# da03/torch-Attention-OCR

Measured on AMD Instinct MI355X. Metric: image-lines/sec (train step), higher is better.
Workload: dtype bf16; 1 GPU; c3: 32x256 crops, batch 256/GPU, VGG-7 + BiLSTM(256) + 2-layer attn decoder, L=24; global_batch=256, per_gpu_batch=256, img=32x256, decoder_steps=24, parallelism=dp1, input_feed=True

## Files before the change

### include/aocr.h

```cpp
#ifndef AOCR_H
#define AOCR_H
#include <stddef.h>
#include <stdint.h>

#ifdef __cplusplus
extern "C" {
#endif

#define AOCR_VERSION 1
#define AOCR_NUM_GROUPS 5
#define AOCR_COMPUTE_F32 0
#define AOCR_COMPUTE_BF16 1

typedef struct aocr_model aocr_model;

typedef struct aocr_config {
  int32_t batch_size;
  int32_t img_h;
  int32_t max_img_w;
  int32_t enc_hidden;
  int32_t enc_layers;
  int32_t dec_layers;
  int32_t vocab;
  int32_t emb;
// ... 66 lines not shown
                     const aocr_trie* trie, int32_t* labels_dev, float* scores_dev,
                     float* gold_scores_dev, float* loss_dev);

int aocr_recognize(aocr_model* m, const float* images_dev, int32_t B, int32_t W, int32_t beam,
                   const aocr_trie* trie, int32_t* labels_dev, float* scores_dev,
                   float* char_logp_dev, float* attn_dev);

int aocr_get_tensor(aocr_model* m, const char* name, const void** ptr_dev, int32_t* ndim, int64_t shape[4]);

#define AOCR_PK_CONV6_FWD 0
#define AOCR_PK_CONV6_WGRAD 1
#define AOCR_PK_CONV1_FWD 2
#define AOCR_PK_CONV1_BWD 3
#define AOCR_PK_BN_FWD 4
#define AOCR_PK_BN_BWD 5
#define AOCR_PK_UNPOOL 6
#define AOCR_PK_ATTN_DCTX 7
#define AOCR_PK_SPLITK 8
#define AOCR_PK_LAST 8
int aocr_profile_kernel(aocr_model* m, int32_t which, int32_t iters, float* ms_per_launch, double* flops_per_launch);

#define AOCR_PROF_OTHER 0
#define AOCR_PROF_CONV_FWD 1
#define AOCR_PROF_CONV_DGRAD 2
#define AOCR_PROF_CONV_WGRAD 3
#define AOCR_PROF_BN 4
#define AOCR_PROF_POOL_CONV1 5
#define AOCR_PROF_ENC_SEQ 6
#define AOCR_PROF_RNN_GEMM 7
#define AOCR_PROF_DEC_FWD 8
#define AOCR_PROF_DEC_BWD 9
#define AOCR_PROF_SGD 10
#define AOCR_PROF_DECODE 11
#define AOCR_PROF_FAMILIES 12
int aocr_profile_enable(aocr_model* m, int32_t on);
int aocr_profile_read(aocr_model* m, float ms[AOCR_PROF_FAMILIES], int32_t* marks);


#define AOCR_GEMM_ACCUMULATE 1
#define AOCR_GEMM_RELU 2
#define AOCR_GEMM_TANH 4
int aocr_gemm(void* stream, int32_t compute, const float* A_dev, int64_t lda, int32_t a_kmajor,
              const float* B_dev, int64_t ldb, int32_t b_kmajor, float* C_dev, int64_t ldc,
              int32_t M, int32_t N, int32_t K, const float* bias_dev, int32_t accumulate);

int aocr_conv2d_forward(void* stream, int32_t compute, const float* x_dev, const float* w_dev, const float* bias_dev,
                        float* y_dev, uint8_t* idx_dev, int32_t B, int32_t H, int32_t W, int32_t Cin, int32_t Cout,
                        int32_t ksize, int32_t pad, int32_t relu, int32_t pool);
int aocr_conv2d_backward_data(void* stream, int32_t compute, const float* dy_dev, const float* w_dev, float* dx_dev,
                              int32_t B, int32_t H, int32_t W, int32_t Cin, int32_t Cout, int32_t ksize, int32_t pad);
int aocr_conv2d_backward_filter(void* stream, int32_t compute, const float* x_dev, const float* dy_dev, float* dw_dev,
                                float* dbias_dev, int32_t B, int32_t H, int32_t W, int32_t Cin, int32_t Cout,
                                int32_t ksize, int32_t pad);
int aocr_unpool_relu_backward(void* stream, const float* dpooled_dev, const float* pooled_dev, const uint8_t* idx_dev,
                              float* dy_dev, int32_t B, int32_t Ho, int32_t Wo, int32_t C, int32_t pool);

int aocr_conv1_forward(void* stream, const float* x_dev, const float* w_dev, const float* bias_dev, float* y_dev,
                       int32_t B, int32_t H, int32_t W);
int aocr_conv1_backward(void* stream, const float* x_dev, const float* w_dev, const float* bias_dev,
                        const float* dy_pooled_dev, float* dw_dev, float* dbias_dev, int32_t B, int32_t H, int32_t W);

#define AOCR_BN_SCRATCH_BYTES (8u << 20)
int aocr_batchnorm_relu_forward(void* stream, const float* x_dev, float* y_dev, const float* weight_dev,
                                const float* bias_dev, float* running_mean_dev, float* running_var_dev,
                                float* save_dev, void* scratch_dev, int64_t rows, int32_t C, int32_t training,
                                int32_t update_running, int32_t tb_rows);
int aocr_batchnorm_relu_backward(void* stream, const float* x_dev, const float* y_dev, const float* dA_dev,
                                 const float* weight_dev, const float* save_dev, float* dx_dev, float* dweight_dev,
                                 float* dbias_dev, void* scratch_dev, int64_t rows, int32_t C, int32_t tb_rows);

int aocr_lstm_cell_forward(void* stream, int32_t compute, const float* x_dev, int32_t in_size, const float* h_prev_dev,
                           const float* c_prev_dev, const float* w_i2h_dev, const float* b_i2h_dev,
                           const float* w_h2h_dev, const float* b_h2h_dev, float* c_dev, float* h_dev,
                           float* gates_dev, int32_t B, int32_t H);
int aocr_lstm_cell_forward_zx(void* stream, int32_t compute, const float* zx_dev, int64_t ldzx, const float* h_prev_dev,
                              const float* c_prev_dev, const float* w_h2h_dev, float* c_dev, float* h_dev, float* gates_dev,
                              int32_t B, int32_t H);
int aocr_lstm_cell_backward(void* stream, const float* dc_dev, const float* dh_dev, const float* gates_dev,
                            const float* c_prev_dev, const float* c_dev, float* dz_dev, float* dc_prev_dev,
                            int32_t B, int32_t H);

int aocr_attention_forward(void* stream, const float* ctx_dev, const float* q_dev, float* a_dev, float* c_dev,
                           int64_t ldc, int32_t B, int32_t T, int32_t Hd);
int aocr_attention_backward(void* stream, const float* ctx_dev, const float* q_dev, const float* a_dev,
                            const float* dc_dev, int64_t lddc, float* ds_dev, float* dq_dev, int32_t B, int32_t T,
                            int32_t Hd);

#define AOCR_PW_ADD 0
#define AOCR_PW_TANH_BWD 1
#define AOCR_PW_RELU_BWD 2
#define AOCR_PW_RELU 3
int aocr_pointwise(void* stream, int32_t op, const float* a_dev, const float* b_dev, float* y_dev, int64_t n);

int aocr_lookup_forward(void* stream, const float* weight_dev, const int32_t* ids_dev, float* out_dev, int32_t n, int32_t E);
int aocr_lookup_backward(void* stream, const float* grad_out_dev, const int32_t* ids_dev, float* grad_weight_dev, int32_t n, int32_t E, int32_t V);

int aocr_logsoftmax_nll(void* stream, const float* logits_dev, int64_t ld, const int32_t* targets_dev, float* logp_dev,
                        float* dlogits_dev, float* nll_rows_dev, int64_t rows, int32_t V, float grad_scale);

int aocr_beam_select(void* stream, const float* logp_dev, const int32_t* prev_tok_dev, float* beam_scores_dev,
                     int32_t* tokens_dev, int32_t* parents_dev, int32_t B, int32_t kin, int32_t kout, int32_t V);

int aocr_beam_select_dict(void* stream, const float* logp_dev, const int32_t* prev_tok_dev, float* beam_scores_dev,
                          int32_t* tokens_dev, int32_t* parents_dev, int32_t B, int32_t kin, int32_t kout, int32_t V,
                          const aocr_trie* trie, const int32_t* loc_in_dev, int32_t* loc_out_dev);

// ... 139 lines not shown
```

### torch-attention-ocr_amd/aocr/_lib.py

```python
from __future__ import annotations

import ctypes as C
import os

import torch

_HERE = os.path.dirname(os.path.abspath(__file__))
LIB_PATH = os.environ.get("AOCR_LIB") or os.path.join(_HERE, "libaocr.so")

NUM_GROUPS = 5
COMPUTE_F32, COMPUTE_BF16 = 0, 1
PROF_FAMILIES = ["other", "conv_fwd", "conv_dgrad", "conv_wgrad", "bn", "pool_conv1", "encoder_seq", "rnn_gemm", "decoder_fwd",
                 "decoder_bwd", "sgd", "decode_chain"]


class AocrError(RuntimeError):
    pass


class TrieDesc(C.Structure):
    _fields_ = [("child_mask_dev", C.c_void_p), ("child_base_dev", C.c_void_p), ("child_dev", C.c_void_p),
                ("n_nodes", C.c_int32), ("n_edges", C.c_int32)]


# ... 54 lines not shown
class Config(C.Structure):
    _fields_ = [(n, C.c_int32) for n in (
        "batch_size", "img_h", "max_img_w", "enc_hidden", "enc_layers", "dec_layers", "vocab", "emb",
        "input_feed", "max_decoder_l", "max_beam", "compute")]


if not os.path.exists(LIB_PATH):
    raise ImportError(
        f"{LIB_PATH} not found: build it with `make -C torch-attention-ocr_amd/csrc` "
        "(or __graft_entry__.build()); there is no CPU fallback for the hot path")

lib = C.CDLL(LIB_PATH)

_vp, _i32, _i64, _f32, _sz = C.c_void_p, C.c_int32, C.c_int64, C.c_float, C.c_size_t
_cfgp = C.POINTER(Config)
ALLREDUCE_FN = C.CFUNCTYPE(C.c_int, _vp, _vp, _i64, _i32, _vp)

SIGNATURES = {
    "aocr_last_error": (C.c_char_p, []),
    "aocr_version": (C.c_int, []),
    "aocr_param_counts": (C.c_int, [_cfgp, C.POINTER(_i64)]),
    "aocr_param_entry": (C.c_int, [_cfgp, _i32, C.c_char_p, C.POINTER(_i32), C.POINTER(_i64), C.POINTER(_i32), C.POINTER(_i64)]),
    "aocr_bn_state_count": (_i64, []),
    "aocr_workspace_bytes": (_sz, [_cfgp]),
    "aocr_model_create": (C.c_int, [_cfgp, _vp, _vp, _vp, _vp, _sz, _vp, C.POINTER(_vp)]),
    "aocr_model_destroy": (C.c_int, [_vp]),
    "aocr_model_set_stream": (C.c_int, [_vp, _vp]),
    "aocr_train_forward_backward": (C.c_int, [_vp, _vp, _vp, _vp, _i32, _i32, _i32, _f32, _vp]),
    "aocr_set_dropout": (C.c_int, [_vp, C.c_double, C.c_uint64, C.c_uint64]),
    "aocr_cluster_status": (C.c_int, [_vp, C.POINTER(_i32)]),
    "aocr_grad_buckets": (C.c_int, [_cfgp, C.POINTER(_i64), C.POINTER(_i64)]),
    "aocr_stream_wait_grads": (C.c_int, [_vp, _i32, _vp]),
    "aocr_comm_unique_id": (C.c_int, [C.c_char_p]),
    "aocr_comm_init_rank": (C.c_int, [_vp, C.c_char_p, _i32, _i32, _i32]),
    "aocr_comm_set_callback": (C.c_int, [_vp, _vp, _vp, _i32, _i32]),
    "aocr_allreduce_grads": (C.c_int, [_vp, _vp]),
    "aocr_comm_destroy": (C.c_int, [_vp]),
    "aocr_comm_exposed_ms": (C.c_int, [_vp, C.POINTER(_f32)]),
    "aocr_comm_info": (C.c_int, [_vp, C.POINTER(_i32), C.POINTER(_i32), C.POINTER(_i32)]),
    "aocr_sgd_step": (C.c_int, [_vp, _f32, _f32, _vp]),
    "aocr_adadelta_step": (C.c_int, [_vp, _f32, _f32, _f32, _vp]),
    "aocr_forward_logits": (C.c_int, [_vp, _vp, _vp, _vp, _i32, _i32, _i32, _i32, _vp, _vp]),
    "aocr_decode": (C.c_int, [_vp, _vp, _vp, _vp, _i32, _i32, _i32, _i32, _vp, _vp, _vp, _vp]),
    "aocr_decode_dict": (C.c_int, [_vp, _vp, _vp, _vp, _i32, _i32, _i32, _i32, _vp, _vp, _vp, _vp, _vp]),
    "aocr_recognize": (C.c_int, [_vp, _vp, _i32, _i32, _i32, _vp, _vp, _vp, _vp, _vp]),
    "aocr_get_tensor": (C.c_int, [_vp, C.c_char_p, C.POINTER(_vp), C.POINTER(_i32), C.POINTER(_i64)]),
    "aocr_profile_kernel": (C.c_int, [_vp, _i32, _i32, C.POINTER(_f32), C.POINTER(C.c_double)]),
    "aocr_profile_enable": (C.c_int, [_vp, _i32]),
    "aocr_profile_read": (C.c_int, [_vp, C.POINTER(_f32), C.POINTER(_i32)]),
    "aocr_gemm": (C.c_int, [_vp, _i32, _vp, _i64, _i32, _vp, _i64, _i32, _vp, _i64, _i32, _i32, _i32, _vp, _i32]),
    "aocr_conv2d_forward": (C.c_int, [_vp, _i32, _vp, _vp, _vp, _vp, _vp] + [_i32] * 9),
    "aocr_conv2d_backward_data": (C.c_int, [_vp, _i32, _vp, _vp, _vp] + [_i32] * 7),
    "aocr_conv2d_backward_filter": (C.c_int, [_vp, _i32, _vp, _vp, _vp, _vp] + [_i32] * 7),
    "aocr_unpool_relu_backward": (C.c_int, [_vp, _vp, _vp, _vp, _vp] + [_i32] * 5),
    "aocr_conv1_forward": (C.c_int, [_vp, _vp, _vp, _vp, _vp, _i32, _i32, _i32]),
    "aocr_conv1_backward": (C.c_int, [_vp, _vp, _vp, _vp, _vp, _vp, _vp, _i32, _i32, _i32]),
    "aocr_batchnorm_relu_forward": (C.c_int, [_vp] * 9 + [_i64, _i32, _i32, _i32, _i32]),
    "aocr_batchnorm_relu_backward": (C.c_int, [_vp] * 10 + [_i64, _i32, _i32]),
    "aocr_lstm_cell_forward": (C.c_int, [_vp, _i32, _vp, _i32] + [_vp] * 9 + [_i32, _i32]),
    "aocr_lstm_cell_forward_zx": (C.c_int, [_vp, _i32, _vp, _i64] + [_vp] * 6 + [_i32, _i32]),
    "aocr_lstm_cell_backward": (C.c_int, [_vp] * 8 + [_i32, _i32]),
    "aocr_attention_forward": (C.c_int, [_vp, _vp, _vp, _vp, _vp, _i64, _i32, _i32, _i32]),
    "aocr_attention_backward": (C.c_int, [_vp, _vp, _vp, _vp, _vp, _i64, _vp, _vp, _i32, _i32, _i32]),
    "aocr_pointwise": (C.c_int, [_vp, _i32, _vp, _vp, _vp, _i64]),
    "aocr_lookup_forward": (C.c_int, [_vp, _vp, _vp, _vp, _i32, _i32]),
    "aocr_lookup_backward": (C.c_int, [_vp, _vp, _vp, _vp, _i32, _i32, _i32]),
    "aocr_logsoftmax_nll": (C.c_int, [_vp, _vp, _i64, _vp, _vp, _vp, _vp, _i64, _i32, _f32]),
    "aocr_beam_select_dict": (C.c_int, [_vp, _vp, _vp, _vp, _vp, _vp, _i32, _i32, _i32, _i32, _vp, _vp, _vp]),
    "aocr_edit_distance": (C.c_int, [_vp, _vp, _vp, _i32, _i32, _vp, _vp]),
    "aocr_lexicon_scratch_bytes": (_sz, [_i32, _i32]),
    "aocr_lexicon_nearest": (C.c_int, [_vp, _vp, _i32, _i32, _vp, _vp, _vp, _vp, _vp]),
    "aocr_preprocess_lines": (C.c_int, [_vp, _vp, _vp, _i32, _i32, _i32, _vp]),
    "aocr_augment_lines": (C.c_int, [_vp, _vp, _vp, _i32, _i32, _i32, C.c_uint64, C.c_uint64, _vp]),
    "aocr_synth_lines": (C.c_int, [_vp, _vp, _vp, _vp, _i32, _i32, _i32, _i32, _vp, _vp, _vp]),
    "aocr_segment_scratch_bytes": (C.c_size_t, [_i32, _i32, _i32]),
    "aocr_segment_page": (C.c_int, [_vp, _vp, C.c_int64, _i32, _i32, _vp, _vp, _i32, _vp, _vp]),
    "aocr_crop_lines": (C.c_int, [_vp, _vp, C.c_int64, _i32, _i32, _vp, _vp, _i32, _i32, _i32, _vp]),
    "aocr_skew_scratch_bytes": (C.c_size_t, [_i32, _i32, _i32]),
    "aocr_estimate_skew": (C.c_int, [_vp, _vp, C.c_int64, _i32, _i32, _vp, _vp, _vp, _vp]),
    "aocr_deskew_page": (C.c_int, [_vp, _vp, C.c_int64, _i32, _i32, _vp, _i32, _i32, _vp, C.c_int64]),
    "aocr_flatten_scratch_bytes": (C.c_size_t, [_i32, _i32, _i32]),
    "aocr_flatten_page": (C.c_int, [_vp, _vp, C.c_int64, _i32, _i32, _vp, _vp, _vp, C.c_int64]),
    "aocr_integral_scratch_bytes": (C.c_size_t, [_i32, _i32]),
    "aocr_ink_integral": (C.c_int, [_vp, _vp, C.c_int64, _i32, _i32, _i32, _i32, _vp, _vp, C.c_int64, _vp]),
    "aocr_layout_scratch_bytes": (C.c_size_t, [_i32, _i32, _i32]),
    "aocr_layout_blocks": (C.c_int, [_vp, _vp, C.c_int64, _i32, _i32, _vp, _vp, _i32, _vp, _vp]),
    "aocr_components_scratch_bytes": (C.c_size_t, [_i32, _i32]),
    "aocr_label_components": (C.c_int, [_vp, _vp, C.c_int64, _i32, _i32, _i32, _i32, _i32, _vp, _vp, C.c_int64, _i32, _vp, _vp]),
    "aocr_clean_scratch_bytes": (C.c_size_t, [_i32, _i32]),
    "aocr_clean_page": (C.c_int, [_vp, _vp, C.c_int64, _i32, _i32, _vp, _vp, _vp, C.c_int64, _vp]),
    "aocr_beam_select": (C.c_int, [_vp, _vp, _vp, _vp, _vp, _vp, _i32, _i32, _i32, _i32]),
}

for _name, (_res, _args) in SIGNATURES.items():
    _fn = getattr(lib, _name)
    _fn.restype = _res
    _fn.argtypes = _args


def last_error() -> str:
    return (lib.aocr_last_error() or b"").decode()


def check(rc: int, what: str = "") -> None:
    if rc != 0:
        raise AocrError(f"{what}: {last_error()}" if what else last_error())
# ... 26 lines not shown
```

### torch-attention-ocr_amd/csrc/capi.hip

```cpp
#include <cmath>
#include <cstdarg>
#include <cstdio>
#include <cstring>
#include <new>
#include <string>
#include "model.h"

using namespace aocr;

static thread_local std::string g_err;
static int fail(const char* fmt, ...) {
  char buf[512]; va_list ap; va_start(ap, fmt); vsnprintf(buf, sizeof buf, fmt, ap); va_end(ap);
  g_err = buf; return 1;
}
static int check_launch(const char* what) {
  hipError_t e = hipGetLastError();
  if (e != hipSuccess) return fail("%s: %s", what, hipGetErrorString(e));
  return 0;
}
#define REQUIRE(cond, ...) do { if (!(cond)) return fail(__VA_ARGS__); } while (0)

static int check_cfg(const aocr_config* c) {
  REQUIRE(c, "config is NULL");
  REQUIRE(c->batch_size >= 1 && c->img_h >= 32 && c->img_h % 16 == 0, "bad batch_size/img_h");
// ... 408 lines not shown
  else if (n == "enc_cs0") { *ptr_dev = m->ecs[0][m->Le - 1]; *ndim = 3; shape[0] = d.T + 2; shape[1] = d.B; shape[2] = m->He; }
  else if (n == "enc_gates0") { *ptr_dev = m->egates[0][m->Le - 1]; *ndim = 3; shape[0] = d.T; shape[1] = d.B; shape[2] = 4 * m->He; }
  else if (n == "cl_err") { *ptr_dev = m->cl_err; *ndim = 1; shape[0] = 8; REQUIRE(m->cl_err, "no cluster kernels in this configuration"); }
  else if (n == "dc_stamps") { REQUIRE(m->dc_xtab, "no decoder cluster kernel in this configuration"); *ptr_dev = m->dc_xtab + (size_t)((d.B + 31) / 32) * 32; *ndim = 1; shape[0] = 32; }
  else if (n == "ds_all") { *ptr_dev = m->ds_all; *ndim = 3; shape[0] = d.L; shape[1] = d.B; shape[2] = d.T; }
  else if (n == "dq_all") { *ptr_dev = m->dq_all; *ndim = 3; shape[0] = d.L; shape[1] = d.B; shape[2] = m->Hd; }
  else if (n == "dcat_all") { *ptr_dev = m->dcat_all; *ndim = 3; shape[0] = d.L; shape[1] = d.B; shape[2] = 2 * m->Hd; }
  else if (n == "dh_rec0" || n == "dh_rec1" || n == "dc_st0" || n == "dc_st1" || n == "dfeed0") {
    const int l = n.back() - '0'; *ptr_dev = n[1] == 'f' ? m->dfeed : (n[1] == 'h' ? m->dh_rec[l] : m->dc_st[l]); *ndim = 2; shape[0] = d.B; shape[1] = m->Hd; }
  else if (n == "dpre_all") { *ptr_dev = m->dpre_all; *ndim = 3; shape[0] = d.L; shape[1] = d.B; shape[2] = m->Hd; }
  else if (n == "dc_bstamps") { REQUIRE(m->dc_xtab, "no decoder cluster kernel in this configuration"); *ptr_dev = m->dc_xtab + (size_t)((d.B + 31) / 32) * 32 + 16; *ndim = 1; shape[0] = 32; }
  else if (n == "dc_times") { REQUIRE(m->cl_err, "no cluster kernels in this configuration"); *ptr_dev = m->cl_err + 16 + 2048; *ndim = 1; shape[0] = 32 * 4 * 16 * 2; }
  else if (n == "g0") {
    const char* e = getenv("AOCR_DBG_STOP"); const int stop = e ? atoi(e) : 0;
    const int64_t cnt = stop == 1 ? (int64_t)d.B * d.T * 512 : (int64_t)d.B * d.H4 * d.W2 * 512;
    if (m->bf16) bf16_to_f32(m->s, m->G0b, m->G0, cnt);
    *ptr_dev = m->G0; *ndim = 4; shape[0] = d.B; shape[1] = stop == 1 ? d.Ho7 : d.H4; shape[2] = stop == 1 ? d.Wo7 : d.W2; shape[3] = 512;
  }
  else return fail("unknown tensor '%s'", name);
  return 0;
}

int aocr_profile_kernel(aocr_model* m, int32_t which, int32_t iters, float* ms_per_launch, double* flops_per_launch) {
  REQUIRE(m && ms_per_launch && flops_per_launch, "NULL argument");
  REQUIRE(m->last_valid, "run a step first");
  REQUIRE(which >= 0 && which <= AOCR_PK_LAST, "unknown kernel id %d", which);
  REQUIRE(iters >= 1, "iters must be >= 1");
  REQUIRE(which < 2 || (m->bf16 && m->last_images && m->last_train), "the HBM-bound kernel ids replay the bf16 TRAINING step: run aocr_train_forward_backward in bf16 mode first");
  const Dims& d = m->last;
  const int64_t n5 = (int64_t)d.B * d.H4 * d.W2;
  REQUIRE((which != 1 && which != AOCR_PK_SPLITK) || (size_t)512 * 4608 <= m->gmax, "kernel id %d sums conv6's filter gradient (512 x 4608 floats) into the gradient-map scratch, which holds %zu floats in this configuration", which, m->gmax);
  REQUIRE((which != AOCR_PK_BN_FWD && which != AOCR_PK_BN_BWD && which != AOCR_PK_UNPOOL) || (n5 % 256 == 0 && n5 / 256 <= 512), "kernel id %d replays conv5's BatchNorm with the epilogue's 256-pixel statistics chunks: %lld pixels are not a multiple of 256 / more than 512 chunks", which, (long long)n5);
  hipEvent_t e0, e1; hipEventCreate(&e0); hipEventCreate(&e1);
  hipStream_t s = m->s; const int B = d.B;
  constexpr size_t SLAB = (size_t)4 << 20;
  double bytes = 0.0;
  const char* const nd = getenv("AOCR_DX16");
  const bool dx16 = (nd && nd[0] == '1') && !getenv("AOCR_BN_PARTIAL_OLD") && !getenv("AOCR_UNPOOL4") && !getenv("AOCR_HALO8") && B * d.H4 * d.W2 % 256 == 0;
  const bf16_t* const g1h = dx16 ? reinterpret_cast<const bf16_t*>(m->G1) : nullptr;
  const double dab = dx16 ? 2.0 : 4.0;
  auto run = [&]() {
    switch (which) {
    case 0:
      if (const char* const pl = getenv("AOCR_PROBE_LAYER")) {
        int bnc = 0, y16 = 0; const int l = atoi(pl);
        if (l == 3) { conv_forward(m->s, m->bf16, m->A2, m->conv[3].w, m->conv[3].b, m->Y3, nullptr, d.B, d.H2, d.W2, 128, 256, 3, 1, 0, 0, m->A2b, m->wb[3], nullptr, 1, nullptr, nullptr, nullptr, (double*)m->bn_scratch, &bnc, &y16); break; }
        if (l == 4) { conv_forward(m->s, m->bf16, m->A3, m->conv[4].w, m->conv[4].b, nullptr, m->idx4, d.B, d.H2, d.W2, 256, 256, 3, 1, 1, 2, m->A3b, m->wb[4], m->A4b, 1); break; }
        if (l == 5) { conv_forward(m->s, m->bf16, m->A4, m->conv[5].w, m->conv[5].b, m->Y5, nullptr, d.B, d.H4, d.W2, 256, 512, 3, 1, 0, 0, m->A4b, m->wb[5], nullptr, 1, nullptr, nullptr, nullptr, (double*)m->bn_scratch, &bnc, &y16); break; }
      }
      conv_forward(m->s, m->bf16, m->A5, m->conv[6].w, m->conv[6].b, m->bf16 ? nullptr : m->A6, m->idx6, d.B, d.H4, d.W2, 512, 512, 3, 1, 1, 2, m->A5b, m->wb[6],
                   m->A6b, 1);
      break;
    case 1:
      conv_backward_filter(m->s, m->bf16, m->A5, m->G0, m->G1, nullptr, d.B, d.H4, d.W2, 512, 512, 3, 1, m->A5b, m->G0b, m->wg_part, m->wg_part_floats, 1);
      break;
    case AOCR_PK_CONV1_FWD:
      conv1_forward(s, m->last_images, m->conv[1].w, m->conv[1].b, nullptr, B, d.H, d.W, m->A1b, m->route1_valid ? m->route1 : nullptr);
      bytes = (double)B * d.H * d.W * 4 + (double)B * d.H1 * d.W1 * 64 * 2 + (m->route1_valid ? (double)conv1_route_elems(B, d.H, d.W) * 2 : 0.0);
      break;
    case AOCR_PK_CONV1_BWD:
      conv1_backward(s, m->last_images, m->conv[1].w, m->conv[1].b, m->G1, m->conv[1].dw, m->conv[1].db, B, d.H, d.W,
                     (size_t)B * d.H1 * d.W1 * 128 >= (size_t)4096 * 640 ? m->G0 + 6 * SLAB : nullptr, nullptr, m->route1_valid ? m->route1 : nullptr);
      bytes = (double)B * d.H * d.W * 4 + (double)B * d.H1 * d.W1 * 64 * 4 + (m->route1_valid ? (double)conv1_route_elems(B, d.H, d.W) * 2 : 0.0);
      break;
    case AOCR_PK_BN_FWD:
      bn_relu_forward(s, m->Y5, nullptr, m->bn[5].w, m->bn[5].b, m->bn[5].rm, m->bn[5].rv, m->bn[5].save, m->bn_scratch, n5, 512, 1, 0, 0, m->A5b, nullptr, (int)(n5 / 256));
      bytes = (double)n5 * 512 * (4 + 2);
      break;
    case AOCR_PK_BN_BWD:
      bn_relu_backward(s, m->Y5, m->A5, m->G1, m->bn[5].w, m->bn[5].save, nullptr, m->bn[5].dw, m->bn[5].db, m->bn_scratch, n5, 512, 0, m->G0b, m->A5b,
                       m->conv[5].db, m->G0 + 2 * SLAB, nullptr, nullptr, nullptr, g1h);
      bytes = (double)n5 * 512 * ((4 + dab + 2) + (4 + dab + 2 + 2));
      break;
    case AOCR_PK_UNPOOL:
      unpool_relu_backward(s, m->G1, m->A6, m->idx6, nullptr, B, d.H4, d.W2, 512, 2, m->G0b, m->conv[6].db, m->G0 + 1 * SLAB, m->A6b, nullptr, g1h);
      bytes = (double)B * d.H6 * d.W2 * 512 * (dab + 1 + 2) + (double)n5 * 512 * 2;
      break;
    case AOCR_PK_ATTN_DCTX:
      attention_dctx(s, m->a_all, m->ds_all, m->dcat_all, 2 * m->Hd, m->q_all, m->dctx, d.L, B, d.T, m->Hd);
      bytes = (double)d.L * B * (2.0 * d.T + 2.0 * m->Hd) * 4 + (double)B * d.T * m->Hd * 4;
      break;
    case AOCR_PK_SPLITK:
      {
        const int ksl = (int)std::min<size_t>(8, m->wg_part_floats / ((size_t)512 * 4608));
        if (ksl >= 1) splitk_reduce(s, m->wg_part, ksl, (size_t)512 * 4608, m->G1);
        bytes = (double)512 * 4608 * 4 * (ksl + 2);
      }
      break;
    }
  };
  run();
  hipEventRecord(e0, m->s);
  for (int i = 0; i < iters; ++i) run();
  hipEventRecord(e1, m->s);
  hipEventSynchronize(e1);
  float ms = 0.f; hipEventElapsedTime(&ms, e0, e1);
  hipEventDestroy(e0); hipEventDestroy(e1);
  *ms_per_launch = ms / iters;
  if (which == 0 && getenv("AOCR_PROBE")) {
    unsigned long long pr[8] = {0}; kprobe_read(pr);
    if (getenv("AOCR_PROBE_LAYER")) for (int k = 1; k >= 0; --k) if (pr[4 * k + 1]) fprintf(stderr, "[aocr] probe: workgroup %d of the tagged launch: start -> K loop %.1f us, K loop %.1f us (%llu cycles = %.2f GHz), whole workgroup (last store acknowledged) %.1f us\n", k ? 17 : 300, pr[4 * k + 2] / 100.0, pr[4 * k + 1] / 100.0, pr[4 * k], pr[4 * k] / (pr[4 * k + 1] * 10.0) , pr[4 * k + 3] / 100.0);
    for (int k = 0; k < 2; ++k) if (pr[4 * k + 1]) fprintf(stderr, "[aocr] probe (%s halo kernel, conv6 forward): K loop of one workgroup %llu shader cycles in %.1f us = %.2f GHz\n", k ? "4-wave" : "8-wave", pr[4 * k], pr[4 * k + 1] / 100.0, pr[4 * k] / (pr[4 * k + 1] * 10.0)), fprintf(stderr, "[aocr]   prologue %.1f us, whole workgroup %.1f us (stores acknowledged)\n", pr[4 * k + 2] / 100.0, pr[4 * k + 3] / 100.0);
  }
  *flops_per_launch = which < 2 ? 2.0 * (double)d.B * d.H4 * d.W2 * 512.0 * (9.0 * 512.0) : bytes;
  return check_launch("aocr_profile_kernel");
}

int aocr_gemm(void* stream, int32_t compute, const float* A_dev, int64_t lda, int32_t a_kmajor, const float* B_dev, int64_t ldb,
              int32_t b_kmajor, float* C_dev, int64_t ldc, int32_t M, int32_t N, int32_t K, const float* bias_dev, int32_t accumulate) {
  REQUIRE(A_dev && B_dev && C_dev && M >= 0 && N >= 0 && K >= 0, "bad gemm arguments");
  REQUIRE((accumulate & ~7) == 0, "unknown gemm flag bits %d", accumulate);
  const int fl = ((accumulate & AOCR_GEMM_ACCUMULATE) ? EP_ACCUM : 0) | ((accumulate & AOCR_GEMM_RELU) ? EP_RELU : 0) | ((accumulate & AOCR_GEMM_TANH) ? EP_TANH : 0);
  REQUIRE(!((fl & EP_ACCUM) && (fl & (EP_RELU | EP_TANH))), "an activation on an accumulating product is not a module of the path");
  int rc = gemm((hipStream_t)stream, compute == AOCR_COMPUTE_BF16, A_dev, lda, a_kmajor != 0, B_dev, ldb, b_kmajor != 0, C_dev, ldc,
                M, N, K, bias_dev, nullptr, fl);
  REQUIRE(rc == 0, "gemm: the (A column-major, B row-major-by-K) combination is not supported");
  return check_launch("aocr_gemm");
}
int aocr_pointwise(void* stream, int32_t op, const float* a_dev, const float* b_dev, float* y_dev, int64_t n) {
  REQUIRE(a_dev && y_dev && n >= 0 && op >= 0 && op <= 3 && (b_dev || op == AOCR_PW_RELU), "bad arguments");
  pointwise((hipStream_t)stream, op, a_dev, b_dev, y_dev, n);
  return check_launch("aocr_pointwise");
}
int aocr_lookup_forward(void* stream, const float* weight_dev, const int32_t* ids_dev, float* out_dev, int32_t n, int32_t E) {
  REQUIRE(weight_dev && ids_dev && out_dev && n >= 0 && E > 0, "bad arguments");
  embedding_gather((hipStream_t)stream, weight_dev, ids_dev, 0, 1, out_dev, 1, n, E);
  return check_launch("aocr_lookup_forward");
}
int aocr_lookup_backward(void* stream, const float* grad_out_dev, const int32_t* ids_dev, float* grad_weight_dev, int32_t n, int32_t E, int32_t V) {
  REQUIRE(grad_out_dev && ids_dev && grad_weight_dev && n >= 0 && E > 0 && E <= 256 && V > 0, "bad arguments");
  embedding_scatter_accum((hipStream_t)stream, grad_out_dev, ids_dev, 0, 1, grad_weight_dev, 1, n, E, V);
  return check_launch("aocr_lookup_backward");
}
int aocr_conv2d_forward(void* stream, int32_t compute, const float* x_dev, const float* w_dev, const float* bias_dev, float* y_dev,
                        uint8_t* idx_dev, int32_t B, int32_t H, int32_t W, int32_t Cin, int32_t Cout, int32_t ksize, int32_t pad,
                        int32_t relu, int32_t pool) {
  REQUIRE(x_dev && w_dev && y_dev, "NULL argument");
  REQUIRE(Cin % 16 == 0 && Cout % 16 == 0, "Cin and Cout must be multiples of 16 (the 1-channel first layer has its own entry point)");
  REQUIRE(pool >= 0 && pool <= 2 && (pool == 0 || idx_dev), "bad pool mode / missing idx");
  conv_forward((hipStream_t)stream, compute == AOCR_COMPUTE_BF16, x_dev, w_dev, bias_dev, y_dev, idx_dev, B, H, W, Cin, Cout, ksize, pad,
               relu, pool);
  return check_launch("aocr_conv2d_forward");
}
int aocr_conv2d_backward_data(void* stream, int32_t compute, const float* dy_dev, const float* w_dev, float* dx_dev, int32_t B, int32_t H,
                              int32_t W, int32_t Cin, int32_t Cout, int32_t ksize, int32_t pad) {
  REQUIRE(dy_dev && w_dev && dx_dev && Cin % 16 == 0 && Cout % 16 == 0, "bad arguments");
  conv_backward_data((hipStream_t)stream, compute == AOCR_COMPUTE_BF16, dy_dev, w_dev, dx_dev, B, H, W, Cin, Cout, ksize, pad);
  return check_launch("aocr_conv2d_backward_data");
}
int aocr_conv2d_backward_filter(void* stream, int32_t compute, const float* x_dev, const float* dy_dev, float* dw_dev, float* dbias_dev,
                                int32_t B, int32_t H, int32_t W, int32_t Cin, int32_t Cout, int32_t ksize, int32_t pad) {
  REQUIRE(x_dev && dy_dev && dw_dev && Cin % 16 == 0 && Cout % 16 == 0, "bad arguments");
  conv_backward_filter((hipStream_t)stream, compute == AOCR_COMPUTE_BF16, x_dev, dy_dev, dw_dev, dbias_dev, B, H, W, Cin, Cout, ksize, pad);
  return check_launch("aocr_conv2d_backward_filter");
}
int aocr_unpool_relu_backward(void* stream, const float* dpooled_dev, const float* pooled_dev, const uint8_t* idx_dev, float* dy_dev,
                              int32_t B, int32_t Ho, int32_t Wo, int32_t C, int32_t pool) {
  REQUIRE(dpooled_dev && pooled_dev && idx_dev && dy_dev && (pool == 1 || pool == 2) && C % 4 == 0, "bad arguments");
  unpool_relu_backward((hipStream_t)stream, dpooled_dev, pooled_dev, idx_dev, dy_dev, B, Ho, Wo, C, pool);
  return check_launch("aocr_unpool_relu_backward");
}
int aocr_conv1_forward(void* stream, const float* x_dev, const float* w_dev, const float* bias_dev, float* y_dev, int32_t B, int32_t H,
                       int32_t W) {
  REQUIRE(x_dev && w_dev && bias_dev && y_dev, "NULL argument");
  conv1_forward((hipStream_t)stream, x_dev, w_dev, bias_dev, y_dev, B, H, W);
  return check_launch("aocr_conv1_forward");
}
int aocr_conv1_backward(void* stream, const float* x_dev, const float* w_dev, const float* bias_dev, const float* dy_pooled_dev,
                        float* dw_dev, float* dbias_dev, int32_t B, int32_t H, int32_t W) {
  REQUIRE(x_dev && w_dev && bias_dev && dy_pooled_dev && dw_dev && dbias_dev, "NULL argument");
  conv1_backward((hipStream_t)stream, x_dev, w_dev, bias_dev, dy_pooled_dev, dw_dev, dbias_dev, B, H, W);
  return check_launch("aocr_conv1_backward");
}
int aocr_batchnorm_relu_forward(void* stream, const float* x_dev, float* y_dev, const float* weight_dev, const float* bias_dev,
                                float* running_mean_dev, float* running_var_dev, float* save_dev, void* scratch_dev, int64_t rows,
                                int32_t C, int32_t training, int32_t update_running, int32_t tb_rows) {
  REQUIRE(x_dev && y_dev && weight_dev && bias_dev && running_mean_dev && running_var_dev && save_dev && scratch_dev, "NULL argument");
  REQUIRE(C % 4 == 0 && C <= 512, "C must be a multiple of 4 and <= 512");
  bn_relu_forward((hipStream_t)stream, x_dev, y_dev, weight_dev, bias_dev, running_mean_dev, running_var_dev, save_dev, scratch_dev, rows, C,
                  training, update_running, tb_rows);
  return check_launch("aocr_batchnorm_relu_forward");
}
int aocr_batchnorm_relu_backward(void* stream, const float* x_dev, const float* y_dev, const float* dA_dev, const float* weight_dev,
                                 const float* save_dev, float* dx_dev, float* dweight_dev, float* dbias_dev, void* scratch_dev,
                                 int64_t rows, int32_t C, int32_t tb_rows) {
  REQUIRE(x_dev && y_dev && dA_dev && weight_dev && save_dev && dx_dev && dweight_dev && dbias_dev && scratch_dev, "NULL argument");
  bn_relu_backward((hipStream_t)stream, x_dev, y_dev, dA_dev, weight_dev, save_dev, dx_dev, dweight_dev, dbias_dev, scratch_dev, rows, C,
                   tb_rows);
  return check_launch("aocr_batchnorm_relu_backward");
}
int aocr_lstm_cell_forward(void* stream, int32_t compute, const float* x_dev, int32_t in_size, const float* h_prev_dev,
                           const float* c_prev_dev, const float* w_i2h_dev, const float* b_i2h_dev, const float* w_h2h_dev,
                           const float* b_h2h_dev, float* c_dev, float* h_dev, float* gates_dev, int32_t B, int32_t H) {
  REQUIRE(x_dev && h_prev_dev && c_prev_dev && w_i2h_dev && b_i2h_dev && w_h2h_dev && b_h2h_dev && c_dev && h_dev, "NULL argument");
  REQUIRE(in_size % 16 == 0 && H % 16 == 0, "in_size and H must be multiples of 16");
  GatesFwdArgs z;
  z.a = make_loadk2(x_dev, in_size, in_size, h_prev_dev, H, H, B);
  z.b = make_loadk2(w_i2h_dev, in_size, in_size, w_h2h_dev, H, H, 4 * H);
  z.K = in_size + H;
  EpGatesFwd& e = z.ep; e.zx = nullptr; e.ldzx = 0; e.b1 = b_i2h_dev; e.b2 = b_h2h_dev; e.c_prev = c_prev_dev; e.ldcp = H;
  e.c_out = c_dev; e.ldc = H; e.h_out = h_dev; e.ldh = H; e.h_out2 = nullptr; e.ldh2 = 0; e.gates = gates_dev; e.ldg = 4 * H; e.M = B; e.H = H;
  launch_small_gates_fwd((hipStream_t)stream, compute == AOCR_COMPUTE_BF16, 1, &z, B, H);
  return check_launch("aocr_lstm_cell_forward");
}
int aocr_lstm_cell_forward_zx(void* stream, int32_t compute, const float* zx_dev, int64_t ldzx, const float* h_prev_dev, const float* c_prev_dev,
                              const float* w_h2h_dev, float* c_dev, float* h_dev, float* gates_dev, int32_t B, int32_t H) {
  REQUIRE(zx_dev && h_prev_dev && c_prev_dev && w_h2h_dev && c_dev && h_dev, "NULL argument");
  REQUIRE(H % 16 == 0 && ldzx >= 4 * (int64_t)H, "H must be a multiple of 16 and ldzx >= 4H");
// ... 347 lines not shown
```

### torch-attention-ocr_amd/csrc/mfma_gemm.h

```cpp
#pragma once
#include <hip/hip_runtime.h>
#include <stdint.h>
#include <type_traits>
#include <utility>

namespace aocr {

typedef float f32x16 __attribute__((ext_vector_type(16)));
typedef float f32x4 __attribute__((ext_vector_type(4)));
typedef __bf16 bf16x8 __attribute__((ext_vector_type(8)));

template <int NV> struct Frag { float v[NV]; };

template <bool BF16> struct Mode {
  static constexpr int NV = BF16 ? 8 : 4;
  static constexpr int CHUNK = BF16 ? 16 : 8;
};


struct LoadK {
  const float* p0; int64_t ld0; int K0;
  const float* p1; int64_t ld1;
  int rows; int K; int vec;
  struct Ctx { const float* b0; const float* b1; bool ok; };
// ... 1834 lines not shown
#pragma unroll
  for (int i = 0; i < 2; ++i)
#pragma unroll
    for (int j = 0; j < 2; ++j)
#pragma unroll
      for (int e = 0; e < 16; ++e) acc[i][j][e] = 0.f;

  const int g = lane >> 4, q = (lane >> 2) & 3, p = lane & 3;
  const int tr_off = (8 * h + q) * TR_PITCH + (16 * (g & 1) + 4 * p) * 2;

  if (nk > 0) { gload(); lwrite(0); }
  __syncthreads();
  for (int kt = 0; kt < nk; ++kt) {
    const int buf = kt & 1;
    if (kt + 1 < nk) gload();
    const unsigned char* la = &lds[buf][0][tr_off + (wm * 64) * 2];
    const unsigned char* lb = &lds[buf][1][tr_off + (wn * 64) * 2];
#pragma unroll
    for (int s = 0; s < 2; ++s) {
      bf16x8 af[2], bf[2];
#pragma unroll
      for (int i = 0; i < 2; ++i) {
        s16x4 a0 = lds_tr_read(la + (16 * s) * TR_PITCH + i * 64), a1 = lds_tr_read(la + (16 * s + 4) * TR_PITCH + i * 64);
        s16x4 b0 = lds_tr_read(lb + (16 * s) * TR_PITCH + i * 64), b1 = lds_tr_read(lb + (16 * s + 4) * TR_PITCH + i * 64);
        typedef short s16x8 __attribute__((ext_vector_type(8)));
        s16x8 av = {a0[0], a0[1], a0[2], a0[3], a1[0], a1[1], a1[2], a1[3]};
        s16x8 bv = {b0[0], b0[1], b0[2], b0[3], b1[0], b1[1], b1[2], b1[3]};
        af[i] = __builtin_bit_cast(bf16x8, av); bf[i] = __builtin_bit_cast(bf16x8, bv);
      }
#pragma unroll
      for (int mi = 0; mi < 2; ++mi)
#pragma unroll
        for (int ni = 0; ni < 2; ++ni)
          acc[mi][ni] = __builtin_amdgcn_mfma_f32_32x32x16_bf16(af[mi], bf[ni], acc[mi][ni], 0, 0, 0);
    }
    if (kt + 1 < nk) lwrite(buf ^ 1);
    __syncthreads();
  }
  const int r = lane & 31;
  const int m0 = m_blk + wm * 64, n0 = n_blk + wn * 64;
#pragma unroll
  for (int mi = 0; mi < 2; ++mi)
#pragma unroll
    for (int qq = 0; qq < 4; ++qq) {
      float v[2][4];
#pragma unroll
      for (int ni = 0; ni < 2; ++ni)
#pragma unroll
        for (int i = 0; i < 4; ++i) v[ni][i] = acc[mi][ni][4 * qq + i];
      ep.template quad<2>(m0 + 32 * mi + 8 * qq + 4 * h, n0 + r, 32, v);
    }
}

template <class EP>
__global__ __launch_bounds__(256, 4) void conv_wgrad_tr_kernel(LoadMNh a, LoadConvXcolh b, EP ep, int K, int kper, int gx, int gy, int gz, float* part, long long pstride) {
  __shared__ __attribute__((aligned(16))) unsigned char lds[2][2][32 * TR_PITCH];
  const int nwg = gx * gy * gz, orig = blockIdx.x;
  const int q8 = nwg >> 3, r8 = nwg & 7, xcd = orig & 7;
  const int lin = (xcd < r8 ? xcd * (q8 + 1) : r8 * (q8 + 1) + (xcd - r8) * q8) + (orig >> 3);
  const int zsp = lin / (gx * gy), bid = lin - zsp * (gx * gy);
  const int kbeg = zsp * kper;
  if (part) { ep.C = part + (size_t)zsp * pstride; ep.flags &= ~8 ; }
  tr_tile(a, b, ep, (bid / gx) * 128, (bid % gx) * 128, kbeg, min(K, kbeg + kper), lds);
}

template <class EP, int ABL = 0>
__global__ __launch_bounds__(512, 1) void conv_wgrad_dma_kernel(LoadMNh a, LoadConvXcolh b, EP ep, int K, int kper, int gx, int gy, const bf16_t* zero, int gz, float* part, long long pstride) {
  __shared__ __attribute__((aligned(1024))) unsigned char lds[4 * 32768];
  const int nwg = gx * gy * gz, orig = blockIdx.x;
  const int q8 = nwg >> 3, r8 = nwg & 7, xcd = orig & 7;
  const int lin = (xcd < r8 ? xcd * (q8 + 1) : r8 * (q8 + 1) + (xcd - r8) * q8) + (orig >> 3);
  const int zsp = lin / (gx * gy), bid = lin - zsp * (gx * gy);
  const int m_blk = (bid / gx) * 256, n_blk = (bid % gx) * 256;
  const int kbeg = zsp * kper, kend = min(K, kbeg + kper);
  if (part) { ep.C = part + (size_t)zsp * pstride; ep.flags &= ~8 ; }
  const int nk = kend > kbeg ? (kend - kbeg + 31) >> 5 : 0;
  const int tid = threadIdx.x, lane = tid & 63, wave = __builtin_amdgcn_readfirstlane(tid >> 6);
  const int h = lane >> 5, wm = wave >> 2, wn = wave & 3;

  int krow[2], chunk[2];
#pragma unroll
  for (int j = 0; j < 2; ++j) {
    krow[j] = 2 * (2 * wave + j) + (lane >> 5);
    const int pos = lane & 31;
    chunk[j] = ((((pos >> 2) ^ (krow[j] & 3)) << 2) | (pos & 3));
  }
  LoadMNh::Ctx8 ca[2]; typename LoadConvXcolh::Ctx8 cb[2]; typename LoadConvXcolh::Cur cur[2]; int ka[2];
#pragma unroll
  for (int j = 0; j < 2; ++j) {
    ca[j] = a.row8(m_blk + 8 * chunk[j]); cb[j] = b.row8(n_blk + 8 * chunk[j]);
    cur[j] = b.seek(cb[j], kbeg + krow[j]); ka[j] = kbeg + krow[j];
  }
  const bf16_t* pa[2]; const int64_t astep = 32 * a.ld;
#pragma unroll
  for (int j = 0; j < 2; ++j) pa[j] = ca[j].b + (int64_t)ka[j] * a.ld;
  unsigned char* const wbase = lds + (2 * wave) * 1024;
  int slot = 0;
  auto issue = [&]() {
#pragma unroll
    for (int j = 0; j < 2; ++j) {
      dma16((ABL & 16) ? zero : dma_select(ca[j].ok && ka[j] < kend, pa[j], zero), wbase + slot * 32768 + j * 1024);
      ka[j] += 32; pa[j] += astep;
    }
#pragma unroll
    for (int j = 0; j < 2; ++j) {
      dma16((ABL & 128) ? zero : b.dsrc8(cb[j], cur[j], kend, zero), wbase + slot * 32768 + 16384 + j * 1024);
      b.advance(cb[j], cur[j]);
    }
    slot = (slot + 1) & 3;
  };

  f32x16 acc[4][2];
#pragma unroll
  for (int i = 0; i < 4; ++i)
#pragma unroll
    for (int j = 0; j < 2; ++j)
#pragma unroll
      for (int e = 0; e < 16; ++e) acc[i][j][e] = 0.f;

  const int g = lane >> 4, q = (lane >> 2) & 3, p4 = lane & 3;
  const unsigned rowoff = (8 * h + q) * 512 + (16 * (g & 1) + 4 * p4) * 2;
  unsigned aseg[4], bseg[2];
#pragma unroll
  for (int i = 0; i < 4; ++i) aseg[i] = rowoff + (((wm * 4 + i) ^ q) << 6);
#pragma unroll
  for (int i = 0; i < 2; ++i) bseg[i] = 16384 + rowoff + (((wn * 2 + i) ^ q) << 6);

  typedef unsigned long long u64;
  typedef u64 u64x2 __attribute__((ext_vector_type(2)));
  const unsigned lbase = (unsigned)(uintptr_t)((__attribute__((address_space(3))) unsigned char*)lds);
#define AOCR_TRR(dst, addr, OFF) asm volatile("ds_read_b64_tr_b16 %0, %1 offset:" #OFF : "=v"(dst) : "v"(addr))
#pragma unroll
  for (int t = 0; t < 3; ++t) issue();
  for (int kt = 0; kt < nk; ++kt) {
    asm volatile("s_waitcnt vmcnt(8)" ::: "memory");
    __builtin_amdgcn_s_barrier();
    const unsigned sl = lbase + (kt & 3) * 32768;
    u64 fa[2][4][2], fb[2][2][2];
#pragma unroll
    for (int i = 0; i < 4; ++i) {
      const unsigned ad = sl + aseg[i];
      if constexpr (ABL & 4) { fa[0][i][0] = fa[0][i][1] = fa[1][i][0] = fa[1][i][1] = ad; continue; }
      AOCR_TRR(fa[0][i][0], ad, 0); AOCR_TRR(fa[0][i][1], ad, 2048); AOCR_TRR(fa[1][i][0], ad, 8192); AOCR_TRR(fa[1][i][1], ad, 10240);
    }
#pragma unroll
    for (int i = 0; i < 2; ++i) {
      const unsigned ad = sl + bseg[i];
      if constexpr (ABL & 4) { fb[0][i][0] = fb[0][i][1] = fb[1][i][0] = fb[1][i][1] = ad; continue; }
      AOCR_TRR(fb[0][i][0], ad, 0); AOCR_TRR(fb[0][i][1], ad, 2048); AOCR_TRR(fb[1][i][0], ad, 8192); AOCR_TRR(fb[1][i][1], ad, 10240);
    }
    if constexpr (!(ABL & 1)) issue();
    asm volatile("s_waitcnt lgkmcnt(0)"
                 : "+v"(fa[0][0][0]), "+v"(fa[0][0][1]), "+v"(fa[0][1][0]), "+v"(fa[0][1][1]), "+v"(fa[0][2][0]), "+v"(fa[0][2][1]),
                   "+v"(fa[0][3][0]), "+v"(fa[0][3][1]), "+v"(fb[0][0][0]), "+v"(fb[0][0][1]), "+v"(fb[0][1][0]), "+v"(fb[0][1][1])
                 :: "memory");
    asm volatile(""
                 : "+v"(fa[1][0][0]), "+v"(fa[1][0][1]), "+v"(fa[1][1][0]), "+v"(fa[1][1][1]), "+v"(fa[1][2][0]), "+v"(fa[1][2][1]),
                   "+v"(fa[1][3][0]), "+v"(fa[1][3][1]), "+v"(fb[1][0][0]), "+v"(fb[1][0][1]), "+v"(fb[1][1][0]), "+v"(fb[1][1][1])
                 :: "memory");
#pragma unroll
    for (int s2 = 0; s2 < 2; ++s2)
#pragma unroll
      for (int mi = 0; mi < 4; ++mi)
#pragma unroll
        for (int ni = 0; ni < 2; ++ni) {
          const u64x2 av = {fa[s2][mi][0], fa[s2][mi][1]}, bv = {fb[s2][ni][0], fb[s2][ni][1]};
          if constexpr (ABL & 2) { acc[mi][ni][0] += (float)(unsigned)(av[0] ^ bv[1]); continue; }
          acc[mi][ni] = __builtin_amdgcn_mfma_f32_32x32x16_bf16(__builtin_bit_cast(bf16x8, av), __builtin_bit_cast(bf16x8, bv), acc[mi][ni], 0, 0, 0);
        }
  }
#undef AOCR_TRR
  asm volatile("s_waitcnt vmcnt(0) lgkmcnt(0)" ::: "memory");
  const int r = lane & 31;
  const int m0 = m_blk + wm * 128, n0 = n_blk + wn * 64;
  if constexpr (std::is_same<EP, EpStore>::value && ABL == 0) {
    if (part && !ep.flags && !ep.bias && !ep.bias2 && !ep.C1 && !ep.Cb && !ep.dg && m_blk + 256 <= ep.M && n_blk + 256 <= ep.N) {
      tile256_store_f32<2, 512>(ep.C, ep.ldc, nullptr, false, acc, lds, m_blk, n_blk, wm, wn, r, h, tid);
      return;
    }
  }
#pragma unroll
  for (int mi = 0; mi < 4; ++mi)
#pragma unroll
    for (int qq = 0; qq < 4; ++qq) {
      float v[2][4];
#pragma unroll
      for (int ni = 0; ni < 2; ++ni)
#pragma unroll
        for (int i = 0; i < 4; ++i) v[ni][i] = acc[mi][ni][4 * qq + i];
      ep.template quad<2>(m0 + 32 * mi + 8 * qq + 4 * h, n0 + r, 32, v);
    }
}

struct WgDmaProblem { const bf16_t* A; const bf16_t* B; long long lda, ldb; int M, N, K, gx, tiles, ks, kper, first; float* part; float* C; long long ldc; long long f4first; };
struct WgDmaArgs { int n, total; long long f4total; WgDmaProblem p[8]; };
template <int UNUSED = 0>
__global__ __launch_bounds__(512, 1) void wgrad_dma_grouped_kernel(WgDmaArgs g, const bf16_t* zero) {
  __shared__ __attribute__((aligned(1024))) unsigned char lds[4 * 32768];
  int pi = 0;
#pragma unroll
  for (int i = 1; i < 8; ++i) if (i < g.n && (int)blockIdx.x >= g.p[i].first) pi = i;
  const WgDmaProblem& P = g.p[pi];
  const int local = blockIdx.x - P.first;
  const int zsp = local / P.tiles, bid = local - zsp * P.tiles;
  const int m_blk = (bid / P.gx) * 256, n_blk = (bid % P.gx) * 256;
  const int kbeg = zsp * P.kper, kend = min(P.K, kbeg + P.kper);
  const int nk = kend > kbeg ? (kend - kbeg + 31) >> 5 : 0;
  const int tid = threadIdx.x, lane = tid & 63, wave = __builtin_amdgcn_readfirstlane(tid >> 6);
  const int h = lane >> 5, wm = wave >> 2, wn = wave & 3;
  const bf16_t* pa[2]; const bf16_t* pb[2]; int ka[2];
#pragma unroll
  for (int j = 0; j < 2; ++j) {
    const int krow = 2 * (2 * wave + j) + (lane >> 5), pos = lane & 31;
    const int chunk = ((((pos >> 2) ^ (krow & 3)) << 2) | (pos & 3));
    ka[j] = kbeg + krow;
    pa[j] = P.A + (long long)ka[j] * P.lda + m_blk + 8 * chunk; pb[j] = P.B + (long long)ka[j] * P.ldb + n_blk + 8 * chunk;
  }
  const long long astep = 32 * P.lda, bstep = 32 * P.ldb;
  unsigned char* const wbase = lds + (2 * wave) * 1024;
  int slot = 0;
  auto issue = [&]() {
#pragma unroll
    for (int j = 0; j < 2; ++j) { dma16(dma_select(ka[j] < kend, pa[j], zero), wbase + slot * 32768 + j * 1024); pa[j] += astep; }
#pragma unroll
    for (int j = 0; j < 2; ++j) { dma16(dma_select(ka[j] < kend, pb[j], zero), wbase + slot * 32768 + 16384 + j * 1024); pb[j] += bstep; ka[j] += 32; }
    slot = (slot + 1) & 3;
  };
  f32x16 acc[4][2];
#pragma unroll
  for (int i = 0; i < 4; ++i)
#pragma unroll
    for (int j = 0; j < 2; ++j)
#pragma unroll
      for (int e = 0; e < 16; ++e) acc[i][j][e] = 0.f;
  const int gq = lane >> 4, q = (lane >> 2) & 3, p4 = lane & 3;
  const unsigned rowoff = (8 * h + q) * 512 + (16 * (gq & 1) + 4 * p4) * 2;
  unsigned aseg[4], bseg[2];
#pragma unroll
  for (int i = 0; i < 4; ++i) aseg[i] = rowoff + (((wm * 4 + i) ^ q) << 6);
#pragma unroll
  for (int i = 0; i < 2; ++i) bseg[i] = 16384 + rowoff + (((wn * 2 + i) ^ q) << 6);
  typedef unsigned long long u64;
  typedef u64 u64x2 __attribute__((ext_vector_type(2)));
  const unsigned lbase = (unsigned)(uintptr_t)((__attribute__((address_space(3))) unsigned char*)lds);
// ... 11 lines not shown
      AOCR_TRR(fa[0][i][0], ad, 0); AOCR_TRR(fa[0][i][1], ad, 2048); AOCR_TRR(fa[1][i][0], ad, 8192); AOCR_TRR(fa[1][i][1], ad, 10240);
    }
#pragma unroll
    for (int i = 0; i < 2; ++i) {
      const unsigned ad = sl + bseg[i];
      AOCR_TRR(fb[0][i][0], ad, 0); AOCR_TRR(fb[0][i][1], ad, 2048); AOCR_TRR(fb[1][i][0], ad, 8192); AOCR_TRR(fb[1][i][1], ad, 10240);
    }
    issue();
    asm volatile("s_waitcnt lgkmcnt(0)"
                 : "+v"(fa[0][0][0]), "+v"(fa[0][0][1]), "+v"(fa[0][1][0]), "+v"(fa[0][1][1]), "+v"(fa[0][2][0]), "+v"(fa[0][2][1]),
                   "+v"(fa[0][3][0]), "+v"(fa[0][3][1]), "+v"(fb[0][0][0]), "+v"(fb[0][0][1]), "+v"(fb[0][1][0]), "+v"(fb[0][1][1])
                 :: "memory");
    asm volatile(""
                 : "+v"(fa[1][0][0]), "+v"(fa[1][0][1]), "+v"(fa[1][1][0]), "+v"(fa[1][1][1]), "+v"(fa[1][2][0]), "+v"(fa[1][2][1]),
                   "+v"(fa[1][3][0]), "+v"(fa[1][3][1]), "+v"(fb[1][0][0]), "+v"(fb[1][0][1]), "+v"(fb[1][1][0]), "+v"(fb[1][1][1])
                 :: "memory");
#pragma unroll
    for (int s2 = 0; s2 < 2; ++s2)
#pragma unroll
      for (int mi = 0; mi < 4; ++mi)
#pragma unroll
        for (int ni = 0; ni < 2; ++ni) {
          const u64x2 av = {fa[s2][mi][0], fa[s2][mi][1]}, bv = {fb[s2][ni][0], fb[s2][ni][1]};
          acc[mi][ni] = __builtin_amdgcn_mfma_f32_32x32x16_bf16(__builtin_bit_cast(bf16x8, av), __builtin_bit_cast(bf16x8, bv), acc[mi][ni], 0, 0, 0);
        }
  }
#undef AOCR_TRR
  asm volatile("s_waitcnt vmcnt(0) lgkmcnt(0)" ::: "memory");
  tile256_store_f32<2, 512>(P.part + (size_t)zsp * P.M * P.N, P.N, nullptr, false, acc, lds, m_blk, n_blk, wm, wn, lane & 31, h, tid);
}
template <int UNUSED = 0>
__global__ __launch_bounds__(256) void wgrad_slab_reduce_kernel(WgDmaArgs g) {
  typedef float f4 __attribute__((ext_vector_type(4)));
  const long long i = (long long)blockIdx.x * 256 + threadIdx.x;
  if (i >= g.f4total) return;
  int pi = 0;
#pragma unroll
  for (int k = 1; k < 8; ++k) if (k < g.n && i >= g.p[k].f4first) pi = k;
  const WgDmaProblem& P = g.p[pi];
  const long long li = i - P.f4first; const int n4 = P.N >> 2; const long long m = li / n4; const int c = (int)(li - m * n4) * 4;
  const size_t mn = (size_t)P.M * P.N;
  const float* src = P.part + (size_t)m * P.N + c;
  f4 acc = {0.f, 0.f, 0.f, 0.f};
  for (int z = 0; z < P.ks; ++z) acc += __builtin_nontemporal_load(reinterpret_cast<const f4*>(src + (size_t)z * mn));
  float* o = P.C + m * P.ldc + c;
  o[0] += acc[0]; o[1] += acc[1]; o[2] += acc[2]; o[3] += acc[3];
}

template <int... I, class F> __device__ __forceinline__ void aocr_static_for_impl(std::integer_sequence<int, I...>, F&& f) { (f(std::integral_constant<int, I>{}), ...); }
template <int N, class F> __device__ __forceinline__ void aocr_static_for(F&& f) { aocr_static_for_impl(std::make_integer_sequence<int, N>{}, f); }
template <int TAG = 0, int MG = 4, bool RG = false, bool IM = false>
__global__ __launch_bounds__(128 * MG, 1)
void conv_wgrad_halo_kernel(const bf16_t* __restrict__ dy, const bf16_t* __restrict__ x, float* __restrict__ part, long long pstride,
                            int nimg, int H, int W, int Cin, int Cout, int gx, int gy, int gz, int segs_per, const bf16_t* zero) {
  constexpr int MT = 64 * MG, NWV = 2 * MG, AROW = MT * 2, RPP = 1024 / AROW, LPR = 64 / RPP;
  constexpr int BOFF = 32 * AROW, SLOT = BOFF + 8192, NS = 6, PW = 34, HPW = 8 / NWV;
  __shared__ __attribute__((aligned(1024))) unsigned char lds[NWV * 20480 > NS * SLOT ? NWV * 20480 : NS * SLOT];
  const int nwg = gx * gy * gz, orig = blockIdx.x;
  const int q8 = nwg >> 3, r8 = nwg & 7, xcd = orig & 7;
  const int lin = (xcd < r8 ? xcd * (q8 + 1) : r8 * (q8 + 1) + (xcd - r8) * q8) + (orig >> 3);
  const int zsp = lin / (gx * gy), bid = lin - zsp * (gx * gy);
  const int m_blk = (bid / gx) * MT, cchunk = bid % gx;
  const int spr = (W + 31) >> 5, S = nimg * H * spr;
  const int s_beg = zsp * segs_per, s_end = min(S, s_beg + segs_per);
  const int nk = s_end > s_beg ? s_end - s_beg : 0;
  const int tid = threadIdx.x, lane = tid & 63, wave = __builtin_amdgcn_readfirstlane(tid >> 6);
  const int h = lane >> 5, mg = wave & (MG - 1), tg = wave / MG;

  const int wrap_px = W - 32 * (spr - 1);
  const int64_t seg0_px = (int64_t)(s_beg / spr) * W + 32 * (s_beg % spr);
  const bf16_t* pa[2]; int akrow[2];
#pragma unroll
  for (int j = 0; j < 2; ++j) {
    const int krow = RPP * (2 * wave + j) + lane / LPR, pos = lane & (LPR - 1);
    const int chunk = ((((pos >> 2) ^ (krow & 3)) << 2) | (pos & 3));
    akrow[j] = krow;
    pa[j] = dy + (seg0_px + krow) * Cout + m_blk + 8 * chunk;
  }
  const int64_t astep = (int64_t)32 * Cout, awrap = (int64_t)wrap_px * Cout;
  bool bin[HPW]; int bry[HPW], bcx[HPW]; const bf16_t* pb[HPW];
#pragma unroll
  for (int j = 0; j < HPW; ++j) {
    const int sl = 64 * (HPW * wave + j) + lane;
    bin[j] = sl < 3 * PW * 4;
    const int hry = sl / (PW * 4), hrem = sl - hry * (PW * 4), hcx = hrem >> 2, hc = hrem & 3;
    bry[j] = hry - 1; bcx[j] = hcx - 1;
    pb[j] = x + (seg0_px + (int64_t)(hry - 1) * W + (hcx - 1)) * Cin + cchunk * 32 + hc * 8;
  }
  const int64_t bstep = (int64_t)32 * Cin, bwrap = (int64_t)wrap_px * Cin;
  int is = s_beg, ixs = s_beg % spr, iy = (s_beg / spr) % H;
  unsigned char* const wA = lds + (2 * wave) * 1024;
  unsigned char* const wB = lds + BOFF + (HPW * wave) * 1024;
  int islot = 0;
  auto issue = [&]() {
    const bool live = is < s_end;
    const int x0 = ixs << 5;
    if constexpr (RG) {
      const bool last = ixs + 1 == spr;
#pragma unroll
      for (int j = 0; j < 2; ++j) { dma16(dma_select(live && x0 + akrow[j] < W, pa[j], zero), wA + islot * SLOT + j * 1024); pa[j] += last ? awrap : astep; }
#pragma unroll
      for (int j = 0; j < HPW; ++j) {
        const bool ok = live && bin[j] && (unsigned)(iy + bry[j]) < (unsigned)H && (unsigned)(x0 + bcx[j]) < (unsigned)W;
        dma16(dma_select(ok, pb[j], zero), wB + islot * SLOT + j * 1024); pb[j] += last ? bwrap : bstep;
      }
      ++is; if (last) { ixs = 0; if (++iy == H) iy = 0; } else ++ixs;
    } else {
// ... 54 lines not shown
            const u64x2 av = {fa[s2][mi][0], fa[s2][mi][1]}, bv = {fb[s2][t][0], fb[s2][t][1]};
            acc[mi][t] = __builtin_amdgcn_mfma_f32_32x32x16_bf16(__builtin_bit_cast(bf16x8, av), __builtin_bit_cast(bf16x8, bv), acc[mi][t], 0, 0, 0);
          }
      };
      if constexpr (!IM) {
        issue();
        asm volatile("s_waitcnt lgkmcnt(0)" : "+v"(fa[0][0][0]), "+v"(fa[0][0][1]), "+v"(fa[0][1][0]), "+v"(fa[0][1][1]), "+v"(fa[1][0][0]), "+v"(fa[1][0][1]), "+v"(fa[1][1][0]), "+v"(fa[1][1][1]) :: "memory");
#pragma unroll
        for (int s2 = 0; s2 < 2; ++s2)
#pragma unroll
          for (int t = 0; t < NTP; ++t) asm volatile("" : "+v"(fb[s2][t][0]), "+v"(fb[s2][t][1]));
        mma_half(std::integral_constant<int, 0>{}); mma_half(std::integral_constant<int, 1>{});
      } else {
        asm volatile("s_waitcnt lgkmcnt(%4)" : "+v"(fa[0][0][0]), "+v"(fa[0][0][1]), "+v"(fa[0][1][0]), "+v"(fa[0][1][1]) : "n"(4 + 2 * NTP) : "memory");
#pragma unroll
        for (int t = 0; t < NTP; ++t) asm volatile("" : "+v"(fb[0][t][0]), "+v"(fb[0][t][1]));
        __builtin_amdgcn_sched_barrier(0);
        mma_half(std::integral_constant<int, 0>{});
        __builtin_amdgcn_sched_barrier(0);
        issue();
        __builtin_amdgcn_sched_barrier(0);
        asm volatile("s_waitcnt lgkmcnt(0)" : "+v"(fa[1][0][0]), "+v"(fa[1][0][1]), "+v"(fa[1][1][0]), "+v"(fa[1][1][1]) :: "memory");
#pragma unroll
        for (int t = 0; t < NTP; ++t) asm volatile("" : "+v"(fb[1][t][0]), "+v"(fb[1][t][1]));
        mma_half(std::integral_constant<int, 1>{});
      }
    }
    asm volatile("s_waitcnt vmcnt(0) lgkmcnt(0)" ::: "memory");
    __syncthreads();
    unsigned char* const wl = lds + wave * 20480;
    constexpr int RP = NTP * 128;
#pragma unroll
    for (int mi = 0; mi < 2; ++mi) {
#pragma unroll
      for (int t = 0; t < NTP; ++t)
#pragma unroll
        for (int qq = 0; qq < 4; ++qq)
#pragma unroll
          for (int i = 0; i < 4; ++i)
            *reinterpret_cast<float*>(wl + (8 * qq + 4 * h + i) * RP + (t * 32 + r) * 4) = acc[mi][t][4 * qq + i];
      asm volatile("s_waitcnt lgkmcnt(0)" ::: "memory");
      const int co0 = m_blk + mg * 64 + mi * 32;
#pragma unroll 4
      for (int it = 0; it < 4 * NTP; ++it) {
        const int idx = it * 64 + lane, row = idx / (8 * NTP), c4 = idx - row * (8 * NTP), t = c4 >> 3, j = c4 & 7;
        const float4 v = *reinterpret_cast<const float4*>(wl + row * RP + c4 * 16);
        *reinterpret_cast<float4*>(slab + (int64_t)(co0 + row) * ldw + (int64_t)(T0 + t) * Cin + cchunk * 32 + j * 4) = v;
      }
      asm volatile("s_waitcnt lgkmcnt(0)" ::: "memory");
    }
  };
  if (tg == 0) body(std::integral_constant<int, 0>{}); else body(std::integral_constant<int, 1>{});
#undef AOCR_TRH
}

template <class AL, class BL, class EP> struct GroupProblem { AL a; BL b; EP ep; int K, kper, gx, ksplit, first; };
template <class AL, class BL, class EP> struct GroupArgs { int n, total; GroupProblem<AL, BL, EP> p[8]; };

template <class AL, class BL, class EP>
__global__ __launch_bounds__(256) void gemm_lds_grouped_kernel(GroupArgs<AL, BL, EP> g) {
  __shared__ __attribute__((aligned(16))) unsigned char lds[2][2][128 * LDS_PITCH];
  int pi = 0;
#pragma unroll
  for (int i = 1; i < 8; ++i) if (i < g.n && (int)blockIdx.x >= g.p[i].first) pi = i;
  const GroupProblem<AL, BL, EP>& P = g.p[pi];
  const int local = blockIdx.x - P.first;
  const int tile = local / P.ksplit, z = local - tile * P.ksplit;
  const int kbeg = z * P.kper;
  lds_tile<32>(P.a, P.b, P.ep, (tile / P.gx) * 128, (tile % P.gx) * 128, kbeg, min(P.K, kbeg + P.kper), lds);
}
template <class EP>
__global__ __launch_bounds__(256, 4) void wgrad_tr_grouped_kernel(GroupArgs<LoadMNh, LoadMNh, EP> g) {
  __shared__ __attribute__((aligned(16))) unsigned char lds[2][2][32 * TR_PITCH];
  int pi = 0;
#pragma unroll
  for (int i = 1; i < 8; ++i) if (i < g.n && (int)blockIdx.x >= g.p[i].first) pi = i;
  const GroupProblem<LoadMNh, LoadMNh, EP>& P = g.p[pi];
  const int local = blockIdx.x - P.first;
  const int tile = local / P.ksplit, z = local - tile * P.ksplit;
  const int kbeg = z * P.kper;
  tr_tile(P.a, P.b, P.ep, (tile / P.gx) * 128, (tile % P.gx) * 128, kbeg, min(P.K, kbeg + P.kper), lds);
}

template <class AL, class BL, class EP> struct SmallArgs { AL a; BL b; EP ep; int K; };

template <bool BF16, int NT, bool GATES, int NW, bool QG, class AL, class BL, class EP>
__device__ __forceinline__ void gemm_small_body(const SmallArgs<AL, BL, EP>& g, int gate_stride, float* red) {
  constexpr int NV = Mode<BF16>::NV, CH = Mode<BF16>::CHUNK;
  const int lane = threadIdx.x & 63, wave = threadIdx.x >> 6;
  const int r = lane & 31, h = lane >> 5;
  const int m0 = blockIdx.y * 32;
  const int n0 = QG ? blockIdx.x * 8 : (GATES ? blockIdx.x * 32 : blockIdx.x * 32 * NT);
  const int K = g.K;

  typename AL::Ctx ca[1]; typename BL::Ctx cb[NT];
  ca[0] = g.a.row(m0 + r);
#pragma unroll
  for (int i = 0; i < NT; ++i) cb[i] = g.b.row(QG ? (r >> 3) * gate_stride + n0 + (r & 7) : (GATES ? i * gate_stride + n0 + r : n0 + 32 * i + r));

  f32x16 acc[1][NT];
#pragma unroll
  for (int j = 0; j < NT; ++j)
#pragma unroll
    for (int e = 0; e < 16; ++e) acc[0][j][e] = 0.f;

  typedef typename FragOf<AL, NV>::type FA; typedef typename FragOf<BL, NV>::type FB;
// ... 332 lines not shown
```

### torch-attention-ocr_amd/csrc/model.h

```cpp
#pragma once
#include <string>
#include <vector>
#include "../../include/aocr.h"
#include "ops.h"

namespace aocr {

constexpr int MAXL = 4;
constexpr int LOGIT_LD = 40;

struct ParamEntry { std::string name; int group; int64_t offset; int ndim; int64_t shape[4]; int64_t numel; };
struct Layout { std::vector<ParamEntry> e; int64_t group_off[AOCR_NUM_GROUPS + 1]; };
Layout build_layout(const aocr_config& c);

struct ConvP { float *w, *b, *dw, *db; int cin, cout, ks, pad; };
struct BnP { float *w, *b, *dw, *db, *rm, *rv, *save; int C; };
struct ShW { const float* w; int64_t ld; int R, C; bf16_t* wb; bf16_t* wtb; float* wtf; };
struct LstmP { float *wi, *bi, *wh, *bh, *dwi, *dbi, *dwh, *dbh; int in; ShW swi, swh; };

struct Arena {
  char* base; size_t off;
  template <class T> T* get(size_t n) {
    off = (off + 255) & ~(size_t)255;
    T* p = base ? reinterpret_cast<T*>(base + off) : nullptr;
    off += n * sizeof(T);
    return p;
  }
};

struct CommState {
  int nranks = 1; bool sync_bn = false; int provider = 0;
  void* rccl = nullptr; void* rccl_bn = nullptr; aocr_allreduce_fn fn = nullptr; void* user = nullptr;
  hipStream_t stream = nullptr; hipEvent_t done = nullptr;
  hipEvent_t wait0 = nullptr, wait1 = nullptr; bool timed = false;
};

struct Dims {
  int B, H, W, L, T;
  int H1, W1, H2, W2, H4, H6, Ho7, Wo7;
};
bool make_dims(const aocr_config& c, int B, int W, int L, Dims& d);

}

struct aocr_model {
  aocr_config cfg;
  hipStream_t s;
  bool bf16;
  float *params, *grads, *bn_state;
  aocr::Layout layout;
  aocr::ConvP conv[8];
  aocr::BnP bn[8];
  aocr::LstmP enc[2][aocr::MAXL], dec[aocr::MAXL];
  float *lookup, *dlookup, *wa, *dwa, *wc, *dwc, *wo, *bo, *dwo, *dbo;
  aocr::ShW swa, swc;
  int He, Hd, Le, Ld, E, V;

  size_t ws_bytes;
  float *A1, *A2, *Y3, *A3, *A4, *Y5, *A5, *A6, *Y7, *X;
  uint8_t *idx2, *idx4, *idx6;
  uint16_t* route1 = nullptr; bool route1_valid = false;
  float *G0, *G1, *dX; size_t gmax = 0;
  aocr::bf16_t *A1b, *A2b, *A3b, *A4b, *A5b, *A6b, *G0b, *G2b = nullptr;
  hipEvent_t cw_map[2] = {nullptr, nullptr}, cw_done[2] = {nullptr, nullptr}, cw_main = nullptr;
  aocr::bf16_t *wb[8], *wtb[8];
  float* wtf[8];
  aocr::bf16_t *Xb, *ehs_b[2][aocr::MAXL], *edz_b[2][aocr::MAXL], *dhs_b[aocr::MAXL], *ddz_b[aocr::MAXL], *out_b, *cat_b, *dpre_b, *dq_b;
  void* bn_scratch; float* bn_save;
  int y16[2] = {0, 0};
  float *ezx[2][aocr::MAXL], *ehs[2][aocr::MAXL], *ecs[2][aocr::MAXL], *egates[2][aocr::MAXL], *edz[2][aocr::MAXL], *edc[2][aocr::MAXL];
  float *edxl[2];
  float *context, *dctx;
  aocr::bf16_t* context_b;
  float* emb_seg = nullptr; int* emb_index = nullptr; bool emb_table = false, tab_valid = false;
  hipEvent_t tab_done = nullptr, zero_done = nullptr, shadow_done = nullptr, shadow2_done = nullptr; bool tab_ready = false, zero_pending = false, shadow_pending = false, shadow2_pending = false;
  int shadow_tiles_conv2 = 0;
  bool proj_fused = false, dout_ready = false;
  float* loss_pending = nullptr;
  hipEvent_t q_go = nullptr, q_done = nullptr; bool q_pending = false;
  hipEvent_t enc_ev = nullptr;
  float *emb_all, *zx1_all, *dhs[aocr::MAXL], *dcs[aocr::MAXL], *dgates[aocr::MAXL], *ddz[aocr::MAXL];
  float *out_all, *cat_all, *q_all, *a_all, *logits, *dlogits, *nll_rows;
  float *dout_proj, *dpre_all, *dcat_all, *ds_all, *dq_all, *demb_all;
  float *dh_rec[aocr::MAXL], *dc_st[aocr::MAXL], *dfeed, *loss_tmp;
  float *bc[2][aocr::MAXL], *bh[2][aocr::MAXL], *bfeed[2], *bc_new[aocr::MAXL], *bh_new[aocr::MAXL];
  aocr::bf16_t *bh_b[2][aocr::MAXL] = {}, *bfeed_b[2] = {}, *bh_new_b[aocr::MAXL] = {}, *bcat_b = nullptr;
  float *bzx1, *bzx_tab, *bq, *ba, *bcat, *bout, *blogits, *blogp, *beam_scores;
  int32_t *hist_tok, *hist_par, *tgt_pad, *tge_pad, *trie_loc[2];
  float *attn_hist = nullptr, *sc_hist = nullptr;
  void* sgd_scratch;
  float* wg_part = nullptr; size_t wg_part_floats = 0;

  std::vector<aocr::ShadowJob> shadow_host;
  aocr::ShadowJob* shadow_dev; int shadow_tiles;
  hipEvent_t grad_ev[4];
  hipStream_t lay_s[aocr::MAXL] = {}; std::vector<hipEvent_t> lay_ev;
  hipStream_t side2 = nullptr; hipEvent_t side2_done = nullptr;
  hipStream_t side = nullptr; hipEvent_t side_go = nullptr, side_done = nullptr; bool side_busy = false;
  int64_t conv5_off;
  aocr::Dims last;
  int last_valid;
  const float* last_images = nullptr; bool last_train = false;
  unsigned long long *cl_xbuf = nullptr, *cl_pbuf = nullptr, *cl_xtab = nullptr; int* cl_err = nullptr; size_t cl_xbytes = 0, cl_pbytes = 0, cl_tbytes = 0; unsigned cl_epoch = 0;
  unsigned long long *dc_xbuf = nullptr, *dc_xtab = nullptr; size_t dc_xbytes = 0, dc_tbytes = 0; aocr::bf16_t* ctxa_b = nullptr; bool ctxa_fresh = false;  bool dgates_il = false; unsigned long long* dc_bxbuf = nullptr; size_t dc_bxbytes = 0; float* dc_pbuf = nullptr;
  double drop_p = 0.0; unsigned long long drop_thr = 0, drop_seed = 0, drop_step = 0; bool drop_on = false;
  float* dhm[aocr::MAXL] = {}; aocr::bf16_t* dhm_b[aocr::MAXL] = {}; float* ehm[2][aocr::MAXL] = {}; aocr::bf16_t* ehm_b[2][aocr::MAXL] = {};
  aocr::CommState comm;
  float* bn_snap = nullptr;
  bool prof_on = false;
  std::vector<hipEvent_t> prof_ev; std::vector<int> prof_tag; size_t prof_n = 0;
};

namespace aocr {
const char* comm_unique_id(char id[128]);
const char* comm_init_rccl(aocr_model* m, const char id[128], int nranks, int rank, int sync_bn);
const char* comm_init_callback(aocr_model* m, aocr_allreduce_fn fn, void* user, int nranks, int sync_bn);
void comm_destroy(aocr_model* m);
int comm_allreduce(aocr_model* m, void* buf, int64_t count, int dtype, hipStream_t stream, int channel);
int comm_allreduce_grads(aocr_model* m, float* loss_dev);
inline bool sync_bn_on(const aocr_model* m) { return m->comm.provider != 0 && m->comm.sync_bn; }
inline bool env_on(const char* name) { const char* e = getenv(name); return e && e[0] == '1'; }
inline bool comm_early_bucket0() { return env_on("AOCR_COMM_EARLY_BUCKET0"); }
inline bool comm_holds_bucket0(const aocr_model* m) { return m->comm.provider != 0 && !comm_early_bucket0(); }
inline int comm_reserved_cus(const aocr_model* m) {
  if (m->comm.provider == 0 || !comm_early_bucket0()) return 0;
  const char* e = getenv("AOCR_COMM_RESERVE_CUS");
  const int n = e ? atoi(e) : 32;
  return n < 0 ? 0 : (n > 128 ? 128 : n);
}
void prof_mark_slow(aocr_model* m, int tag);
inline void prof_mark(aocr_model* m, int tag) { if (m->prof_on) prof_mark_slow(m, tag); }
void step_prologue(aocr_model* m, size_t grad_bytes);
void build_shadow_jobs(aocr_model* m);
int model_carve(aocr_model* m, void* base, size_t bytes);
void cnn_forward(aocr_model* m, const float* images, const Dims& d, int training, int update_running);
void encoder_forward(aocr_model* m, const Dims& d);
void decoder_tf_forward(aocr_model* m, const Dims& d, const int32_t* tgt, int64_t st, int64_t sb, bool keep_gates);
void loss_and_dlogits(aocr_model* m, const Dims& d, const int32_t* tge, int64_t st, int64_t sb, float grad_scale, bool want_grad,
                      float* loss_dev);
void backward_all(aocr_model* m, const float* images, const int32_t* tgt, const Dims& d);
void decode_beam(aocr_model* m, const Dims& d, const int32_t* tgt, int beam, int32_t* labels, float* scores,
                 const aocr_trie* trie = nullptr, float* attn_hist = nullptr, float* sc_hist = nullptr);
}
```

### torch-attention-ocr_amd/csrc/model.hip

```cpp
#include "model.h"
#include <cmath>
#include <cstdio>
#include <cstring>
#include <cstdlib>

namespace aocr {

static void add_entry(Layout& L, int64_t& off, const std::string& name, int group, std::initializer_list<int64_t> shape) {
  ParamEntry e; e.name = name; e.group = group; e.offset = off; e.ndim = (int)shape.size(); e.numel = 1;
  int i = 0; for (int64_t v : shape) { e.shape[i++] = v; e.numel *= v; }
  for (; i < 4; ++i) e.shape[i] = 1;
  off += e.numel; L.e.push_back(e);
}
Layout build_layout(const aocr_config& c) {
  Layout L; int64_t off = 0;
  const int He = c.enc_hidden, Hd = 2 * He;
  static const int convs[7][4] = {{1, 64, 3, 1}, {64, 128, 3, 1}, {128, 256, 3, 1}, {256, 256, 3, 1},
                                  {256, 512, 3, 1}, {512, 512, 3, 1}, {512, 512, 2, 0}};
  L.group_off[0] = 0;
  for (int i = 0; i < 7; ++i) {
    char nm[64];
    snprintf(nm, 64, "cnn.conv%d.w", i + 1); add_entry(L, off, nm, 0, {convs[i][1], convs[i][2], convs[i][2], convs[i][0]});
    snprintf(nm, 64, "cnn.conv%d.b", i + 1); add_entry(L, off, nm, 0, {convs[i][1]});
    if (i == 2 || i == 4 || i == 6) {
// ... 81 lines not shown
    for (int l = 0; l < m->Ld; ++l) { sh(m->dec[l].swi, 4 * Hd, Hd); sh(m->dec[l].swh, 4 * Hd, Hd); }
    sh(m->swa, Hd, Hd); sh(m->swc, Hd, 2 * Hd);
  }
  m->bn_scratch = a.get<char>(bn_scratch_bytes(512)); m->bn_save = a.get<float>(3 * 2 * 512);
  for (int dir = 0; dir < 2; ++dir) {
    for (int l = 0; l < m->Le; ++l) {
      m->ezx[dir][l] = a.get<float>(T * B * 4 * He); m->ehs[dir][l] = a.get<float>((T + 2) * B * He);
      m->ecs[dir][l] = a.get<float>((T + 2) * B * He); m->egates[dir][l] = a.get<float>(T * B * 4 * He);
      m->edz[dir][l] = a.get<float>(T * B * 4 * He);
    }
    for (int l = 0; l < m->Le; ++l) m->edc[dir][l] = a.get<float>(B * He);
    m->edxl[dir] = a.get<float>(T * B * He);
  }
  m->context = a.get<float>(B * T * Hd); m->dctx = a.get<float>(B * T * Hd);
  m->context_b = m->bf16 ? a.get<bf16_t>(B * T * Hd) : nullptr;
  {
    auto hb = [&](size_t n) { return m->bf16 ? a.get<bf16_t>(n) : (bf16_t*)nullptr; };
    m->Xb = hb(T * B * 512);
    for (int dir = 0; dir < 2; ++dir) for (int l = 0; l < m->Le; ++l) { m->ehs_b[dir][l] = hb((T + 2) * B * He); m->edz_b[dir][l] = hb(T * B * 4 * He); }
    for (int l = 0; l < m->Ld; ++l) { m->dhs_b[l] = hb((L + 1) * B * Hd); m->ddz_b[l] = hb(L * B * 4 * Hd); }
    m->out_b = hb((L + 1) * B * Hd); m->cat_b = hb(L * B * 2 * Hd); m->dpre_b = hb(L * B * Hd); m->dq_b = hb(L * B * Hd);
  }
  m->emb_all = a.get<float>(L * B * E); m->zx1_all = a.get<float>(L * B * 4 * Hd); m->emb_seg = a.get<float>((size_t)m->V * 4 * Hd); m->emb_index = a.get<int>(segsum_index_ints((size_t)L * B, m->V));
  for (int l = 0; l < m->Ld; ++l) {
    m->dhs[l] = a.get<float>((L + 1) * B * Hd); m->dcs[l] = a.get<float>((L + 1) * B * Hd);
    m->dgates[l] = a.get<float>(L * B * 4 * Hd); m->ddz[l] = a.get<float>(L * B * 4 * Hd);
    m->dh_rec[l] = a.get<float>(B * Hd); m->dc_st[l] = a.get<float>(B * Hd);
  }
  m->out_all = a.get<float>((L + 1) * B * Hd); m->cat_all = a.get<float>(L * B * 2 * Hd);
  m->q_all = a.get<float>(L * B * Hd); m->a_all = a.get<float>(L * B * T);
  m->logits = a.get<float>(L * B * LOGIT_LD); m->dlogits = a.get<float>(L * B * LOGIT_LD); m->nll_rows = a.get<float>(L * B);
  m->dout_proj = a.get<float>(L * B * Hd); m->dpre_all = a.get<float>(L * B * Hd); m->dcat_all = a.get<float>(L * B * 2 * Hd);
  m->ds_all = a.get<float>(L * B * T); m->dq_all = a.get<float>(L * B * Hd); m->demb_all = a.get<float>(L * B * E);
  m->dfeed = a.get<float>(B * Hd); m->loss_tmp = a.get<float>(64);
  for (int p = 0; p < 2; ++p) {
    for (int l = 0; l < m->Ld; ++l) { m->bc[p][l] = a.get<float>(R * Hd); m->bh[p][l] = a.get<float>(R * Hd); }
    m->bfeed[p] = a.get<float>(R * Hd);
  }
  for (int l = 0; l < m->Ld; ++l) { m->bc_new[l] = a.get<float>(R * Hd); m->bh_new[l] = a.get<float>(R * Hd); }
  if (m->bf16) {
    for (int p = 0; p < 2; ++p) { for (int l = 0; l < m->Ld; ++l) m->bh_b[p][l] = a.get<bf16_t>(R * Hd); m->bfeed_b[p] = a.get<bf16_t>(R * Hd); }
    for (int l = 0; l < m->Ld; ++l) m->bh_new_b[l] = a.get<bf16_t>(R * Hd);
    m->bcat_b = a.get<bf16_t>(R * 2 * Hd);
  }
  m->bzx1 = a.get<float>(R * 4 * Hd); m->bzx_tab = a.get<float>((size_t)m->V * 4 * Hd); m->bq = a.get<float>(R * Hd); m->ba = a.get<float>(R * T);
  m->bcat = a.get<float>(R * 2 * Hd); m->bout = a.get<float>(R * Hd); m->blogits = a.get<float>(R * LOGIT_LD);
  m->blogp = a.get<float>(R * m->V); m->beam_scores = a.get<float>(R);
  m->hist_tok = a.get<int32_t>(L * R); m->hist_par = a.get<int32_t>(L * R);
  m->attn_hist = a.get<float>(L * R * T); m->sc_hist = a.get<float>(L * R);
  m->tgt_pad = a.get<int32_t>(B * L); m->tge_pad = a.get<int32_t>(B * L);
  m->trie_loc[0] = a.get<int32_t>(R); m->trie_loc[1] = a.get<int32_t>(R);
  m->sgd_scratch = a.get<char>(sgd_scratch_bytes());
  m->wg_part_floats = m->bf16 ? (size_t)20 << 20 : 0;       m->wg_part = m->wg_part_floats ? a.get<float>(m->wg_part_floats) : nullptr;
  if (m->bf16 && He % 64 == 0 && He <= 512) {
    m->cl_xbytes = m->Le * enc_cluster_xbuf_bytes((int)B, (int)He); m->cl_pbytes = m->Le * enc_cluster_pbuf_bytes((int)B, (int)He);
    m->cl_xbuf = a.get<unsigned long long>(m->cl_xbytes / 8); m->cl_pbuf = a.get<unsigned long long>(m->cl_pbytes / 8);
    m->cl_tbytes = ((size_t)m->Le * 4 * ((B + 15) / 16) * 8 + 64) * 8;
    m->cl_xtab = a.get<unsigned long long>(m->cl_tbytes / 8);
    m->cl_err = a.get<int>(16 + 256 * 8 + 4096);
    m->bn_snap = a.get<float>(2 * (256 + 512 + 512));
    if (Hd == 1024) m->ctxa_b = a.get<bf16_t>(B * T * Hd);
    if (Hd == 512 && m->Ld == 2 && m->cfg.input_feed) {
      m->dc_xbytes = dec_cluster_xbuf_bytes((int)B); m->dc_tbytes = dec_cluster_xtab_bytes((int)std::max<size_t>(B, 32 * (size_t)dec_chain_beam_group_cap()));
      m->dc_xbuf = a.get<unsigned long long>(m->dc_xbytes / 8); m->dc_xtab = a.get<unsigned long long>(m->dc_tbytes / 8);
      m->ctxa_b = a.get<bf16_t>(B * T * Hd);
      m->dc_bxbytes = dec_cluster_bwd_xbuf_bytes((int)B); m->dc_bxbuf = a.get<unsigned long long>(m->dc_bxbytes / 8);
      m->dc_pbuf = a.get<float>(dec_cluster_pbuf_bytes((int)std::max<size_t>(B, 32 * (size_t)dec_chain_beam_group_cap())) / 4);
    }
  }
  for (int l = 0; l + 1 < m->Ld; ++l) { m->dhm[l] = a.get<float>(L * B * Hd); m->dhm_b[l] = m->bf16 ? a.get<bf16_t>(L * B * Hd) : nullptr; }
  for (int dir = 0; dir < 2; ++dir) for (int l = 0; l + 1 < m->Le; ++l) { m->ehm[dir][l] = a.get<float>(T * B * He); m->ehm_b[dir][l] = m->bf16 ? a.get<bf16_t>(T * B * He) : nullptr; }
  m->shadow_dev = m->bf16 ? a.get<ShadowJob>(128) : nullptr;
  m->ws_bytes = a.off + 256;
  if (base && a.off > bytes) return -1;
  return 0;
}

void build_shadow_jobs(aocr_model* m) {
  m->shadow_host.clear(); m->shadow_tiles = 0;
  if (!m->bf16 || !m->shadow_dev) return;
  auto add = [&](const float* w, bf16_t* wb, bf16_t* wtb, int64_t ld, int64_t ldb, int64_t ldt, int R, int C) {
    ShadowJob j{w, wb, wtb, ld, ldb, ldt, R, C, m->shadow_tiles, cdiv(C, 32)};
    m->shadow_tiles += cdiv(C, 32) * cdiv(R, 32);
    m->shadow_host.push_back(j);
  };
  auto up = [&](const ShW& w) { if (w.wb) add(w.w, w.wb, w.wtb, w.ld, w.C, w.R, w.R, w.C); };
  auto conv_jobs = [&](int i) {
    const ConvP& c = m->conv[i]; const int KK = c.ks * c.ks;
    for (int tap = 0; tap < KK; ++tap)
      add(c.w + (size_t)tap * c.cin, m->wb[i] + (size_t)tap * c.cin, m->wtb[i] + (size_t)tap * c.cout, (int64_t)KK * c.cin,
          (int64_t)KK * c.cin, (int64_t)KK * c.cout, c.cout, c.cin);
  };
  conv_jobs(2);
  m->shadow_tiles_conv2 = m->shadow_tiles;
  for (int dir = 0; dir < 2; ++dir) for (int l = 0; l < m->Le; ++l) { up(m->enc[dir][l].swh); up(m->enc[dir][l].swi); }
  for (int l = 0; l < m->Ld; ++l) { if (l > 0 || m->cfg.input_feed) up(m->dec[l].swi); up(m->dec[l].swh); }
  up(m->swa); up(m->swc);
  for (int i = 3; i <= 7; ++i) conv_jobs(i);
  if (m->shadow_host.size() > 128) { m->shadow_host.clear(); m->shadow_tiles = 0; m->shadow_tiles_conv2 = 0; }
}
static void refresh_rnn_shadows(aocr_model* m, hipStream_t st = nullptr) {
  if (!st) st = m->s;
  auto up = [&](const ShW& w) {
    if (w.wb) weight_shadows(st, w.w, w.ld, w.R, w.C, w.wb, w.wtb);
    else if (w.wtf) transpose_f32(st, w.w, w.ld, w.R, w.C, w.wtf);
  };
// ... 101 lines not shown
  prof_mark(m, AOCR_PROF_POOL_CONV1); conv1_forward(s, images, m->conv[1].w, m->conv[1].b, bf ? nullptr : m->A1, B, d.H, d.W, m->A1b, training ? m->route1 : nullptr);
  m->route1_valid = training;
  if (m->shadow_pending && m->shadow2_pending) { hipStreamWaitEvent(s, m->shadow2_done, 0); m->shadow2_pending = false; }
  else if (m->shadow_pending) { hipStreamWaitEvent(s, m->shadow_done, 0); m->shadow_pending = false; }
  prof_mark(m, AOCR_PROF_CONV_FWD); conv_forward(s, bf, m->A1, m->conv[2].w, m->conv[2].b, bf ? nullptr : m->A2, m->idx2, B, d.H1, d.W1, 64, 128, 3, 1, 1, 1, m->A1b, m->wb[2], m->A2b);
  if (m->shadow_pending) { hipStreamWaitEvent(s, m->shadow_done, 0); m->shadow_pending = false; }
  const bool fold = bf && !training && !getenv("AOCR_NO_BN_FOLD");
  if (fold) {
    prof_mark(m, AOCR_PROF_BN); bn_eval_prepare(s, m->bn[3].rm, m->bn[3].rv, m->bn[3].save, 256);
    prof_mark(m, AOCR_PROF_CONV_FWD); conv_forward(s, bf, m->A2, m->conv[3].w, m->conv[3].b, nullptr, nullptr, B, d.H2, d.W2, 128, 256, 3, 1, 0, 0, m->A2b, m->wb[3], m->A3b, 0,
                                                   m->bn[3].save, m->bn[3].w, m->bn[3].b);
  } else {
  int bnc = 0;
  prof_mark(m, AOCR_PROF_CONV_FWD); conv_forward(s, bf, m->A2, m->conv[3].w, m->conv[3].b, m->Y3, nullptr, B, d.H2, d.W2, 128, 256, 3, 1, 0, 0, m->A2b, m->wb[3], nullptr, 0,
                                                 nullptr, nullptr, nullptr, training ? (double*)m->bn_scratch : nullptr, &bnc, &m->y16[0]);
  prof_mark(m, AOCR_PROF_BN); bn_relu_forward(s, m->Y3, bf ? nullptr : m->A3, m->bn[3].w, m->bn[3].b, m->bn[3].rm, m->bn[3].rv, m->bn[3].save, m->bn_scratch,
                  (int64_t)B * d.H2 * d.W2, 256, training, update_running, 0, m->A3b, bsync, bnc, m->y16[0] ? reinterpret_cast<const bf16_t*>(m->Y3) : nullptr);
  }
  prof_mark(m, AOCR_PROF_CONV_FWD); conv_forward(s, bf, m->A3, m->conv[4].w, m->conv[4].b, bf ? nullptr : m->A4, m->idx4, B, d.H2, d.W2, 256, 256, 3, 1, 1, 2, m->A3b, m->wb[4], m->A4b);
  if (fold) {
    prof_mark(m, AOCR_PROF_BN); bn_eval_prepare(s, m->bn[5].rm, m->bn[5].rv, m->bn[5].save, 512);
    prof_mark(m, AOCR_PROF_CONV_FWD); conv_forward(s, bf, m->A4, m->conv[5].w, m->conv[5].b, nullptr, nullptr, B, d.H4, d.W2, 256, 512, 3, 1, 0, 0, m->A4b, m->wb[5], m->A5b, 0,
                                                   m->bn[5].save, m->bn[5].w, m->bn[5].b);
  } else {
  int bnc = 0;
  prof_mark(m, AOCR_PROF_CONV_FWD); conv_forward(s, bf, m->A4, m->conv[5].w, m->conv[5].b, m->Y5, nullptr, B, d.H4, d.W2, 256, 512, 3, 1, 0, 0, m->A4b, m->wb[5], nullptr, 0,
                                                 nullptr, nullptr, nullptr, training ? (double*)m->bn_scratch : nullptr, &bnc, &m->y16[1]);
  prof_mark(m, AOCR_PROF_BN); bn_relu_forward(s, m->Y5, bf ? nullptr : m->A5, m->bn[5].w, m->bn[5].b, m->bn[5].rm, m->bn[5].rv, m->bn[5].save, m->bn_scratch,
                  (int64_t)B * d.H4 * d.W2, 512, training, update_running, 0, m->A5b, bsync, bnc, m->y16[1] ? reinterpret_cast<const bf16_t*>(m->Y5) : nullptr);
  }
  prof_mark(m, AOCR_PROF_CONV_FWD); conv_forward(s, bf, m->A5, m->conv[6].w, m->conv[6].b, bf ? nullptr : m->A6, m->idx6, B, d.H4, d.W2, 512, 512, 3, 1, 1, 2, m->A5b, m->wb[6], m->A6b);
  prof_mark(m, AOCR_PROF_CONV_FWD); conv_forward(s, bf, m->A6, m->conv[7].w, m->conv[7].b, m->Y7, nullptr, B, d.H6, d.W2, 512, 512, 2, 0, 0, 0, m->A6b, m->wb[7], nullptr);
  prof_mark(m, AOCR_PROF_BN); bn_relu_forward(s, m->Y7, m->X, m->bn[7].w, m->bn[7].b, m->bn[7].rm, m->bn[7].rv, m->bn[7].save, m->bn_scratch,
                  (int64_t)B * d.T, 512, training, update_running, B, m->Xb, bsync);
}

static bool cnn_wgrad_on_side(aocr_model* m) {
  auto evok = [](hipEvent_t& e) { return e || hipEventCreateWithFlags(&e, hipEventDisableTiming) == hipSuccess; };
  return m->bf16 && m->G2b && !getenv("AOCR_DBG_STOP") && !m->prof_on && m->side && m->side_done && !getenv("AOCR_NO_SIDE_WGRAD") && !env_on("AOCR_NO_CNN_WGRAD_SIDE") &&
         evok(m->cw_map[0]) && evok(m->cw_map[1]) && evok(m->cw_done[0]) && evok(m->cw_done[1]) && evok(m->cw_main);
}

static void cnn_backward(aocr_model* m, const float* images, const Dims& d) {
  hipStream_t s = m->s; const bool bf = m->bf16; const int B = d.B;
  const BnSync bsync_v{bn_sync_allreduce, m}; const BnSync* bsync = sync_bn_on(m) ? &bsync_v : nullptr;
  float *G0 = m->G0, *G1 = m->G1;
  bf16_t* Gb[2] = {m->G0b, m->G2b}; int gp = 0;
  const char* dbg_stop = getenv("AOCR_DBG_STOP");
  const int stop = dbg_stop ? atoi(dbg_stop) : 0;
  const bool ws = !stop && cnn_wgrad_on_side(m);
  hipStream_t sw = ws ? m->side : s;
  const bool wg_after = ws && env_on("AOCR_CNN_WGRAD_AFTER_DGRAD");
  if (!ws) Gb[1] = Gb[0];
  auto map_ready = [&]() { if (ws) { hipEventRecord(m->cw_map[gp], s); hipStreamWaitEvent(sw, m->cw_map[gp], 0); } };
  auto wgrad_done = [&]() { if (ws) hipEventRecord(m->cw_done[gp], sw); };
  auto next_map = [&]() { if (ws) { gp ^= 1; hipStreamWaitEvent(s, m->cw_done[gp], 0); } };
  int bnbc = 0;
  int g16 = 0; const bf16_t* const G1h = reinterpret_cast<const bf16_t*>(G1);
  constexpr size_t SLAB = (size_t)4 << 20;
  ColsumJobs cj; cj.n = 0; cj.total = 0;
  ColsumJobs* defer = (bf && m->gmax >= 8 * SLAB && !getenv("AOCR_NO_COLSUM_DEFER")) ? &cj : nullptr;
  auto slab = [&](int k) { return defer ? G0 + (size_t)k * SLAB : G0; };
  prof_mark(m, AOCR_PROF_BN); bn_relu_backward(s, m->Y7, m->X, m->dX, m->bn[7].w, m->bn[7].save, bf ? nullptr : G0, m->bn[7].dw, m->bn[7].db, m->bn_scratch,
                   (int64_t)B * d.T, 512, B, Gb[gp], bf ? m->Xb : nullptr, bf ? m->conv[7].db : nullptr, bf ? slab(0) : nullptr, bsync, defer);
  if (stop == 1) { if (defer) colsum_flush(s, cj); return; }
  { auto W = [&]() { prof_mark(m, AOCR_PROF_CONV_WGRAD); conv_backward_filter(sw, bf, m->A6, G0, m->conv[7].dw, bf ? nullptr : m->conv[7].db, B, d.H6, d.W2, 512, 512, 2, 0, m->A6b, Gb[gp], m->wg_part, m->wg_part_floats); };
    auto D = [&]() { prof_mark(m, AOCR_PROF_CONV_DGRAD); conv_backward_data(s, bf, G0, m->conv[7].w, G1, B, d.H6, d.W2, 512, 512, 2, 0, Gb[gp], m->wtb[7], m->wtf[7], bf ? &g16 : nullptr); };
    if (wg_after) { D(); map_ready(); W(); wgrad_done(); } else { map_ready(); W(); wgrad_done(); D(); } }
  next_map(); prof_mark(m, AOCR_PROF_POOL_CONV1); unpool_relu_backward(s, G1, m->A6, m->idx6, bf ? nullptr : G0, B, d.H4, d.W2, 512, 2, Gb[gp], bf ? m->conv[6].db : nullptr, bf ? slab(1) : nullptr, bf ? m->A6b : nullptr, defer, g16 ? G1h : nullptr);
  if (stop == 2) { if (defer) colsum_flush(s, cj); return; }
  { auto W = [&]() { prof_mark(m, AOCR_PROF_CONV_WGRAD); conv_backward_filter(sw, bf, m->A5, G0, m->conv[6].dw, bf ? nullptr : m->conv[6].db, B, d.H4, d.W2, 512, 512, 3, 1, m->A5b, Gb[gp], m->wg_part, m->wg_part_floats); };
    auto D = [&]() { prof_mark(m, AOCR_PROF_CONV_DGRAD); { const BnBwdFuse bf5{m->Y5, m->A5b, m->bn[5].save, (double*)m->bn_scratch}; conv_backward_data(s, bf, G0, m->conv[6].w, G1, B, d.H4, d.W2, 512, 512, 3, 1, Gb[gp], m->wtb[6], m->wtf[6], bf ? &g16 : nullptr, (bf && !m->y16[1]) ? &bf5 : nullptr, &bnbc); } };
    if (wg_after) { D(); map_ready(); W(); wgrad_done(); } else { map_ready(); W(); wgrad_done(); D(); } }
  next_map(); prof_mark(m, AOCR_PROF_BN); bn_relu_backward(s, m->Y5, m->A5, G1, m->bn[5].w, m->bn[5].save, bf ? nullptr : G0, m->bn[5].dw, m->bn[5].db, m->bn_scratch,
                   (int64_t)B * d.H4 * d.W2, 512, 0, Gb[gp], bf ? m->A5b : nullptr, bf ? m->conv[5].db : nullptr, bf ? slab(2) : nullptr, bsync, defer, m->y16[1] ? reinterpret_cast<const bf16_t*>(m->Y5) : nullptr, g16 ? G1h : nullptr, bnbc); bnbc = 0;
  { auto W = [&]() { prof_mark(m, AOCR_PROF_CONV_WGRAD); conv_backward_filter(sw, bf, m->A4, G0, m->conv[5].dw, bf ? nullptr : m->conv[5].db, B, d.H4, d.W2, 256, 512, 3, 1, m->A4b, Gb[gp], m->wg_part, m->wg_part_floats); };
    auto D = [&]() { prof_mark(m, AOCR_PROF_CONV_DGRAD); conv_backward_data(s, bf, G0, m->conv[5].w, G1, B, d.H4, d.W2, 256, 512, 3, 1, Gb[gp], m->wtb[5], m->wtf[5], bf ? &g16 : nullptr); };
    if (wg_after) { D(); map_ready(); W(); wgrad_done(); } else { map_ready(); W(); wgrad_done(); }
  if (defer) colsum_flush(s, cj);
  if (ws) { hipEventRecord(m->cw_main, s); hipStreamWaitEvent(sw, m->cw_main, 0); hipEventRecord(m->grad_ev[2], sw); }
  else hipEventRecord(m->grad_ev[2], s);
    if (!wg_after) D(); }
  next_map(); prof_mark(m, AOCR_PROF_POOL_CONV1); unpool_relu_backward(s, G1, m->A4, m->idx4, bf ? nullptr : G0, B, d.H2, d.W2, 256, 2, Gb[gp], bf ? m->conv[4].db : nullptr, bf ? slab(3) : nullptr, bf ? m->A4b : nullptr, defer, g16 ? G1h : nullptr);
  { auto W = [&]() { prof_mark(m, AOCR_PROF_CONV_WGRAD); conv_backward_filter(sw, bf, m->A3, G0, m->conv[4].dw, bf ? nullptr : m->conv[4].db, B, d.H2, d.W2, 256, 256, 3, 1, m->A3b, Gb[gp], m->wg_part, m->wg_part_floats); };
    auto D = [&]() { prof_mark(m, AOCR_PROF_CONV_DGRAD); { const BnBwdFuse bf3{m->Y3, m->A3b, m->bn[3].save, (double*)m->bn_scratch}; conv_backward_data(s, bf, G0, m->conv[4].w, G1, B, d.H2, d.W2, 256, 256, 3, 1, Gb[gp], m->wtb[4], m->wtf[4], bf ? &g16 : nullptr, (bf && !m->y16[0]) ? &bf3 : nullptr, &bnbc); } };
    if (wg_after) { D(); map_ready(); W(); wgrad_done(); } else { map_ready(); W(); wgrad_done(); D(); } }
  next_map(); prof_mark(m, AOCR_PROF_BN); bn_relu_backward(s, m->Y3, m->A3, G1, m->bn[3].w, m->bn[3].save, bf ? nullptr : G0, m->bn[3].dw, m->bn[3].db, m->bn_scratch,
                   (int64_t)B * d.H2 * d.W2, 256, 0, Gb[gp], bf ? m->A3b : nullptr, bf ? m->conv[3].db : nullptr, bf ? slab(4) : nullptr, bsync, defer, m->y16[0] ? reinterpret_cast<const bf16_t*>(m->Y3) : nullptr, g16 ? G1h : nullptr, bnbc); bnbc = 0;
  { auto W = [&]() { prof_mark(m, AOCR_PROF_CONV_WGRAD); conv_backward_filter(sw, bf, m->A2, G0, m->conv[3].dw, bf ? nullptr : m->conv[3].db, B, d.H2, d.W2, 128, 256, 3, 1, m->A2b, Gb[gp], m->wg_part, m->wg_part_floats); };
    auto D = [&]() { prof_mark(m, AOCR_PROF_CONV_DGRAD); conv_backward_data(s, bf, G0, m->conv[3].w, G1, B, d.H2, d.W2, 128, 256, 3, 1, Gb[gp], m->wtb[3], m->wtf[3]); };
    if (wg_after) { D(); map_ready(); W(); wgrad_done(); } else { map_ready(); W(); wgrad_done(); D(); } }
  next_map(); prof_mark(m, AOCR_PROF_POOL_CONV1); unpool_relu_backward(s, G1, m->A2, m->idx2, bf ? nullptr : G0, B, d.H1, d.W1, 128, 1, Gb[gp], bf ? m->conv[2].db : nullptr, bf ? slab(5) : nullptr, bf ? m->A2b : nullptr, defer);
  { auto W = [&]() { prof_mark(m, AOCR_PROF_CONV_WGRAD); conv_backward_filter(sw, bf, m->A1, G0, m->conv[2].dw, bf ? nullptr : m->conv[2].db, B, d.H1, d.W1, 64, 128, 3, 1, m->A1b, Gb[gp], m->wg_part, m->wg_part_floats); };
    auto D = [&]() { prof_mark(m, AOCR_PROF_CONV_DGRAD); conv_backward_data(s, bf, G0, m->conv[2].w, G1, B, d.H1, d.W1, 64, 128, 3, 1, Gb[gp], m->wtb[2], m->wtf[2]); };
    if (wg_after) { D(); map_ready(); W(); wgrad_done(); } else { map_ready(); W(); wgrad_done(); D(); } }
  prof_mark(m, AOCR_PROF_POOL_CONV1); conv1_backward(s, images, m->conv[1].w, m->conv[1].b, G1, m->conv[1].dw, m->conv[1].db, B, d.H, d.W,
                 (size_t)B * d.H1 * d.W1 * 128 >= (size_t)4096 * 640 ? slab(6) : nullptr, defer,
                 m->route1_valid && !getenv("AOCR_CONV1_RECOMPUTE") ? m->route1 : nullptr);
  if (defer) colsum_flush(s, cj);
  if (ws) { hipEventRecord(m->side_done, sw); hipStreamWaitEvent(s, m->side_done, 0); }
}

static bool seq_kernels_ok(const aocr_model* m, int B) {
  if (!m->bf16 || !m->ehs_b[0][0] || !m->enc[0][0].swh.wb) return false;
  const char* e = getenv("AOCR_NO_SEQ");
  if (e && e[0] == '1') return false;
  static const int cus = [] { int n = 0, dev = 0; (void)hipGetDevice(&dev); (void)hipDeviceGetAttribute(&n, hipDeviceAttributeMultiprocessorCount, dev); return n; }();
  return enc_seq_supported(B, m->He, cus);
}

static bool cluster_ok(const aocr_model* m, int B, int T, int& G, int& RT, int& groups) {
  if (!m->bf16 || !m->cl_xbuf || !m->ehs_b[0][0] || !m->enc[0][0].swh.wb || !m->edz_b[0][0]) return false;
  const char* e = getenv("AOCR_NO_CLUSTER");
  if (e && e[0] == '1') return false;
  e = getenv("AOCR_NO_SEQ");
  if (e && e[0] == '1') return false;
  static const int cus = [] { int n = 0, dev = 0; (void)hipGetDevice(&dev); (void)hipDeviceGetAttribute(&n, hipDeviceAttributeMultiprocessorCount, dev); return n; }();
  return enc_cluster_plan(B, m->He, T, cus - comm_reserved_cus(m), G, RT, groups);
}
static unsigned next_epoch(aocr_model* m) {
  if (++m->cl_epoch >= (1u << 20)) {
    hipMemsetAsync(m->cl_xbuf, 0, m->cl_xbytes, m->s); hipMemsetAsync(m->cl_pbuf, 0, m->cl_pbytes, m->s); m->cl_epoch = 1;
    hipMemsetAsync(m->cl_xtab, 0, m->cl_tbytes, m->s);
    if (m->dc_xbuf) { hipMemsetAsync(m->dc_xbuf, 0, m->dc_xbytes, m->s); hipMemsetAsync(m->dc_xtab, 0, m->dc_tbytes, m->s); hipMemsetAsync(m->dc_bxbuf, 0, m->dc_bxbytes, m->s); }
  }
  return m->cl_epoch;
}

static DropSpec drop_site(const aocr_model* m, int site, long long off) {
  DropSpec d;
  if (!m->drop_on) return d;
  const unsigned long long stream = m->drop_step * 64ull + (unsigned long long)site;
  d.base = splitmix64_(m->drop_seed ^ (stream * 0xD1342543DE82EF95ull)); d.thr = m->drop_thr; d.scale = (float)(1.0 / (1.0 - m->drop_p)); d.off = off;
  return d;
}

static int layer_pipe_chunks(const aocr_model* m, int T, int G, int groups) {
  if (m->Le < 2 || m->prof_on || getenv("AOCR_NO_LAYER_PIPE")) return 0;
  static const int cus = [] { int n = 0, dev = 0; (void)hipGetDevice(&dev); (void)hipDeviceGetAttribute(&n, hipDeviceAttributeMultiprocessorCount, dev); return n; }();
  if (2 * groups * G * m->Le > cus) return 0;
  int C = std::min(8, T / 48);
  if (const char* e = getenv("AOCR_LAYER_PIPE_CHUNKS")) C = std::min(atoi(e), T);
  return C >= 2 ? C : 0;
}
static bool layer_pipe_streams(aocr_model* m, int n_events) {
  for (int l = 1; l < m->Le; ++l)
    if (!m->lay_s[l] && hipStreamCreateWithFlags(&m->lay_s[l], hipStreamNonBlocking) != hipSuccess) { m->lay_s[l] = nullptr; return false; }
  while ((int)m->lay_ev.size() < n_events) {
    hipEvent_t e; if (hipEventCreateWithFlags(&e, hipEventDisableTiming) != hipSuccess) return false;
    m->lay_ev.push_back(e);
  }
  return true;
}
static void reserve_epochs(aocr_model* m, unsigned n) { if (m->cl_epoch + n + 1 >= (1u << 20)) { m->cl_epoch = (1u << 20); (void)next_epoch(m); } }

static void encoder_forward_pipe(aocr_model* m, const Dims& d, int C, int clG, int clRT, int clGroups) {
  hipStream_t s0 = m->s;
  const int B = d.B, T = d.T, He = m->He, Hd = m->Hd, Le = m->Le;
  const size_t slot = (size_t)B * He;
  for (int l = 0; l < Le; ++l) {
    ZeroList zl;
    for (int dir = 0; dir < 2; ++dir) {
      zl.add(m->ehs[dir][l], slot * sizeof(float)); zl.add(m->ehs[dir][l] + (size_t)(T + 1) * slot, slot * sizeof(float));
      zl.add(m->ecs[dir][l], slot * sizeof(float)); zl.add(m->ecs[dir][l] + (size_t)(T + 1) * slot, slot * sizeof(float));
      zl.add(m->ehs_b[dir][l], slot * sizeof(bf16_t)); zl.add(m->ehs_b[dir][l] + (size_t)(T + 1) * slot, slot * sizeof(bf16_t));
    }
    zero_many(s0, zl);
  }
  for (int dir = 0; dir < 2; ++dir) {
    const LstmP& p = m->enc[dir][0];
    gemm_hh(s0, m->Xb, p.in, p.swi.wb, p.in, m->ezx[dir][0], 4 * He, T * B, 4 * He, p.in, p.bi, p.bh, 0);
  }
  reserve_epochs(m, (unsigned)(C * Le));
  hipEvent_t* ev = m->lay_ev.data();
  hipEventRecord(ev[Le * C], s0);
  for (int l = 1; l < Le; ++l) hipStreamWaitEvent(m->lay_s[l], ev[Le * C], 0);
  const int Tc = (T + C - 1) / C;
  for (int c = 0; c < C; ++c) {
    const int it0 = c * Tc, it1 = std::min(T, it0 + Tc);
    if (it0 >= it1) break;
    for (int l = 0; l < Le; ++l) {
      hipStream_t sl = l == 0 ? s0 : m->lay_s[l];
      if (l > 0) {
        hipStreamWaitEvent(sl, ev[(l - 1) * C + c], 0);
        for (int dir = 0; dir < 2; ++dir) {
          const LstmP& p = m->enc[dir][l];
          const int t_lo = dir ? T - it1 : it0, n = it1 - it0;
          const bf16_t* xinb = m->ehs_b[dir][l - 1] + (size_t)(t_lo + 1) * slot;
          if (m->drop_on) {
            dropout_apply_b(sl, xinb, m->ehm[dir][l - 1] + (size_t)t_lo * slot, m->ehm_b[dir][l - 1] + (size_t)t_lo * slot, (int64_t)n * slot,
                            drop_site(m, (dir ? 48 : 32) + l + 1, (long long)t_lo * (long long)slot));
            xinb = m->ehm_b[dir][l - 1] + (size_t)t_lo * slot;
          }
          gemm_hh(sl, xinb, p.in, p.swi.wb, p.in, m->ezx[dir][l] + (size_t)t_lo * B * 4 * He, 4 * He, n * B, 4 * He, p.in, p.bi, p.bh, 0);
        }
      }
      const bool top = l == Le - 1;
      EncClFwdArgs a; a.B = B; a.T = T; a.He = He; a.Hd = Hd; a.groups = clGroups; a.epoch = next_epoch(m); a.xbuf = m->cl_xbuf; a.err = m->cl_err; a.xtab = m->cl_xtab;
      a.it0 = it0; a.it1 = it1; a.gslot = l * 2 * clGroups;
      for (int dir = 0; dir < 2; ++dir) {
        EncSeqDir& e = a.d[dir];
        e.w = m->enc[dir][l].swh.wb; e.zx = m->ezx[dir][l]; e.hs = m->ehs[dir][l]; e.cs = m->ecs[dir][l]; e.hsb = m->ehs_b[dir][l];
        e.gates = m->egates[dir][l]; e.ctx = top ? m->context + dir * He : nullptr; e.reverse = dir;
      }
      enc_cluster_forward(sl, a, clG, clRT, comm_reserved_cus(m), Le);
      if (!top) hipEventRecord(ev[l * C + c], sl);
    }
  }
  for (int l = 1; l < Le; ++l) { hipEventRecord(ev[Le * C + l], m->lay_s[l]); hipStreamWaitEvent(s0, ev[Le * C + l], 0); }
}

void encoder_forward(aocr_model* m, const Dims& d) {
  m->ctxa_fresh = false;
  hipStream_t s = m->s; const bool bf = m->bf16;
  const int B = d.B, T = d.T, He = m->He, Hd = m->Hd;
  const size_t slot = (size_t)B * He;
  int clG = 0, clRT = 0, clGroups = 0;
  const bool cluster = cluster_ok(m, B, T, clG, clRT, clGroups);
  const int pipeC = cluster ? layer_pipe_chunks(m, T, clG, clGroups) : 0;
  if (pipeC && layer_pipe_streams(m, (m->Le + 1) * pipeC + m->Le + 1)) {
    if (getenv("AOCR_TRACE")) fprintf(stderr, "[aocr] encoder forward: cluster kernels, layer wavefront of %d chunks\n", pipeC);
    encoder_forward_pipe(m, d, pipeC, clG, clRT, clGroups);
    if (m->context_b) copy2d_bf16(s, m->context, Hd, m->context_b, Hd, B * T, Hd);
    return;
  }
  for (int l = 0; l < m->Le; ++l) {
    ZeroList zl;
    for (int dir = 0; dir < 2; ++dir) {
      const LstmP& p = m->enc[dir][l];
      const float* xin = l == 0 ? m->X : m->ehs[dir][l - 1] + slot;
      const bf16_t* xinb = l == 0 ? m->Xb : (m->ehs_b[dir][l - 1] ? m->ehs_b[dir][l - 1] + slot : nullptr);
      prof_mark(m, AOCR_PROF_RNN_GEMM);
      if (l > 0 && m->drop_on) {
        if (cluster && xinb)
          dropout_apply_b(s, xinb, m->ehm[dir][l - 1], m->ehm_b[dir][l - 1], (int64_t)T * B * He, drop_site(m, (dir ? 48 : 32) + l + 1, 0));
        else
        dropout_apply(s, xin, m->ehm[dir][l - 1], m->ehm_b[dir][l - 1], (int64_t)T * B * He, drop_site(m, (dir ? 48 : 32) + l + 1, 0));
        xin = m->ehm[dir][l - 1]; xinb = m->ehm_b[dir][l - 1];
      }
      if (bf && xinb && p.swi.wb && p.in % 32 == 0)
        gemm_hh(s, xinb, p.in, p.swi.wb, p.in, m->ezx[dir][l], 4 * He, T * B, 4 * He, p.in, p.bi, p.bh, 0);
      else
        gemm(s, bf, xin, p.in, true, p.wi, p.in, true, m->ezx[dir][l], 4 * He, T * B, 4 * He, p.in, p.bi, p.bh, 0);
      zl.add(m->ehs[dir][l], slot * sizeof(float)); zl.add(m->ehs[dir][l] + (size_t)(T + 1) * slot, slot * sizeof(float));
      zl.add(m->ecs[dir][l], slot * sizeof(float)); zl.add(m->ecs[dir][l] + (size_t)(T + 1) * slot, slot * sizeof(float));
      if (m->ehs_b[dir][l]) {
        zl.add(m->ehs_b[dir][l], slot * sizeof(bf16_t)); zl.add(m->ehs_b[dir][l] + (size_t)(T + 1) * slot, slot * sizeof(bf16_t));
      }
    }
    prof_mark(m, AOCR_PROF_OTHER);
    zero_many(s, zl);
    prof_mark(m, AOCR_PROF_ENC_SEQ);
    const bool top = l == m->Le - 1;
    if (getenv("AOCR_TRACE")) fprintf(stderr, "[aocr] encoder layer %d forward: %s kernels\n", l, cluster ? "cluster" : seq_kernels_ok(m, B) ? "whole-sequence" : "per-step");
    if (cluster) {
      EncClFwdArgs a; a.B = B; a.T = T; a.He = He; a.Hd = Hd; a.groups = clGroups; a.epoch = next_epoch(m); a.xbuf = m->cl_xbuf; a.err = m->cl_err; a.xtab = m->cl_xtab;
      for (int dir = 0; dir < 2; ++dir) {
        EncSeqDir& e = a.d[dir];
        e.w = m->enc[dir][l].swh.wb; e.zx = m->ezx[dir][l]; e.hs = m->ehs[dir][l]; e.cs = m->ecs[dir][l]; e.hsb = m->ehs_b[dir][l];
        e.gates = m->egates[dir][l]; e.ctx = top ? m->context + dir * He : nullptr; e.reverse = dir;
      }
      enc_cluster_forward(s, a, clG, clRT, comm_reserved_cus(m));
      continue;
    }
    if (seq_kernels_ok(m, B)) {
      EncSeqFwdArgs a; a.B = B; a.T = T; a.He = He; a.Hd = Hd;
      for (int dir = 0; dir < 2; ++dir) {
        EncSeqDir& e = a.d[dir];
        e.w = m->enc[dir][l].swh.wb; e.zx = m->ezx[dir][l]; e.hs = m->ehs[dir][l]; e.cs = m->ecs[dir][l]; e.hsb = m->ehs_b[dir][l];
        e.gates = m->egates[dir][l]; e.ctx = top ? m->context + dir * He : nullptr; e.reverse = dir;
      }
      enc_seq_forward(s, a);
      continue;
    }
    for (int i = 0; i < T; ++i) {
      LoadK la[2]; LoadKh2 lah[2]; EpGatesFwd ee[2]; const ShW* w0[2]; const ShW* w1[2] = {nullptr, nullptr};
      for (int dir = 0; dir < 2; ++dir) {
        const LstmP& p = m->enc[dir][l];
        const int t = dir == 0 ? i : T - 1 - i;
        const int prev = dir == 0 ? t : t + 2;
        float* hs = m->ehs[dir][l]; float* cs = m->ecs[dir][l];
        la[dir] = make_loadk(hs + prev * slot, He, B, He);
        lah[dir] = make_loadkh(m->ehs_b[dir][l] ? m->ehs_b[dir][l] + prev * slot : nullptr, He, B, He);
        w0[dir] = &p.swh;
        EpGatesFwd& e = ee[dir];
        e.zx = m->ezx[dir][l] + (size_t)t * B * 4 * He; e.ldzx = 4 * He; e.b1 = nullptr; e.b2 = nullptr;
        e.c_prev = cs + prev * slot; e.ldcp = He;
        e.c_out = cs + (size_t)(t + 1) * slot; e.ldc = He; e.h_out = hs + (size_t)(t + 1) * slot; e.ldh = He;
        e.h_out2 = top ? m->context + (size_t)t * Hd + dir * He : nullptr; e.ldh2 = (int64_t)T * Hd;
        e.gates = m->egates[dir][l] + (size_t)t * B * 4 * He; e.ldg = 4 * He; e.M = B; e.H = He;
        if (m->ehs_b[dir][l]) { e.hb = m->ehs_b[dir][l] + (size_t)(t + 1) * slot; e.ldhb = He; }
      }
      run_gates_fwd(m, 2, la, w0, w1, ee, B, He, lah);
    }
  }
  prof_mark(m, AOCR_PROF_OTHER);
  if (m->context_b) copy2d_bf16(s, m->context, Hd, m->context_b, Hd, B * T, Hd);
}

static void encoder_backward_pipe(aocr_model* m, const Dims& d, int C, int clG, int clRT, int clGroups) {
  hipStream_t s0 = m->s;
  const int B = d.B, T = d.T, He = m->He, Hd = m->Hd, Le = m->Le;
  const size_t slot = (size_t)B * He;
// ... 691 lines not shown
```

### torch-attention-ocr_amd/csrc/ops.h

```cpp
#pragma once
#include <hip/hip_runtime.h>
#include <stdint.h>
#include "aocr.h"
#include "epilogues.h"
#include "mfma_gemm.h"

namespace aocr {

inline int cdiv(int64_t a, int64_t b) { return (int)((a + b - 1) / b); }

inline LoadK make_loadk(const float* p, int64_t ld, int rows, int K) {
  LoadK l; l.p0 = p; l.ld0 = ld; l.K0 = K; l.p1 = nullptr; l.ld1 = 0; l.rows = rows; l.K = K;
  l.vec = (((uintptr_t)p & 15) == 0) && (ld % 4 == 0);
  return l;
}
inline LoadK make_loadk2(const float* p0, int64_t ld0, int K0, const float* p1, int64_t ld1, int K1, int rows) {
  LoadK l; l.p0 = p0; l.ld0 = ld0; l.K0 = K0; l.p1 = p1; l.ld1 = ld1; l.rows = rows; l.K = K0 + K1;
  l.vec = (((uintptr_t)p0 & 15) == 0) && (ld0 % 4 == 0) && (((uintptr_t)p1 & 15) == 0) && (ld1 % 4 == 0) && (K0 % 16 == 0);
  return l;
}
inline LoadMN make_loadmn(const float* p, int64_t ld, int rows, int K) {
  LoadMN l; l.p = p; l.ld = ld; l.rows = rows; l.K = K;
  l.vec = (((uintptr_t)p & 15) == 0) && (ld % 4 == 0);
  return l;
// ... 25 lines not shown
typedef SmallArgs<LoadK, LoadKh2, EpStore> SmallArgsH;
typedef SmallArgs<LoadK, LoadKh2, EpGatesBwd> GatesBwdArgsH;
typedef SmallArgs<LoadKh2, LoadKh2, EpGatesFwd> GatesFwdArgsHH;
typedef SmallArgs<LoadKh2, LoadKh2, EpStore> SmallArgsHH;
typedef SmallArgs<LoadKh2, LoadKh2, EpGatesBwd> GatesBwdArgsHH;
void launch_small_gates_fwd_hh(hipStream_t s, int nz, const GatesFwdArgsHH* z, int M, int H);
bool big_step_store(hipStream_t s, const LoadKh2& a, const LoadKh2& b, const EpStore& ep, int M, int N);
bool big_step_gates_fwd(hipStream_t s, const LoadKh2& a, const LoadKh2& b, const EpGatesFwd& ep, int M, int H, float* zbuf, size_t zbuf_floats);
void launch_small_hh(hipStream_t s, int nz, const SmallArgsHH* z, int M, int N);
void launch_small_gates_bwd_hh(hipStream_t s, int nz, const GatesBwdArgsHH* z, int M, int H);
void launch_small_gates_fwd_h(hipStream_t s, int nz, const GatesFwdArgsH* z, int M, int H);
void launch_small_h(hipStream_t s, int nz, const SmallArgsH* z, int M, int N);
void launch_small_gates_bwd_h(hipStream_t s, int nz, const GatesBwdArgsH* z, int M, int H);
inline LoadKh2 make_loadkh(const bf16_t* p, int64_t ld, int rows, int K) {
  LoadKh2 l; l.p0 = p; l.ld0 = ld; l.K0 = K; l.p1 = nullptr; l.ld1 = 0; l.rows = rows; l.K = K; return l;
}
inline LoadKh2 make_loadkh2(const bf16_t* p0, int64_t ld0, int K0, const bf16_t* p1, int64_t ld1, int K1, int rows) {
  LoadKh2 l; l.p0 = p0; l.ld0 = ld0; l.K0 = K0; l.p1 = p1; l.ld1 = ld1; l.rows = rows; l.K = K0 + K1; return l;
}
void weight_shadows(hipStream_t s, const float* w, int64_t ld, int R, int C, bf16_t* wb, bf16_t* wtb);
void transpose_f32(hipStream_t s, const float* w, int64_t ld, int R, int C, float* wt);
void conv_weight_transpose_f32(hipStream_t s, const float* w, float* wt, int Cout, int KK, int Cin);

bool project_loss_ok(int rows, int V, int Hd);
void project_loss(hipStream_t s, const float* out, int64_t ldo, const float* wo, const float* bo, float* logits, float* dlogits, int64_t ld, float* nll, float* dout,
                  const int32_t* tgt, int64_t st, int64_t sb, int Bt, int rows, int V, int Hd, float scale);
int gemm(hipStream_t s, bool bf16, const float* A, int64_t lda, bool a_kmajor, const float* B, int64_t ldb, bool b_kmajor,
          float* C, int64_t ldc, int M, int N, int K, const float* bias, const float* bias2, int flags);

struct WGradProblem { const float* A; int64_t lda; const float* B; int64_t ldb; float* C; int64_t ldc; int M, N, K;
                      const bf16_t* Ab = nullptr; const bf16_t* Bb = nullptr; };
void grouped_wgrad(hipStream_t s, bool bf16, const WGradProblem* p, int n, float* part = nullptr, size_t part_floats = 0);
void kprobe_read(unsigned long long out[8]);

bool gemm_hh_cat(hipStream_t s, const bf16_t* A0, const bf16_t* A1, int64_t lda, const bf16_t* B0, const bf16_t* B1, int64_t ldb, float* C, int64_t ldc, int M, int N, int K0, int K1);
void gemm_hh(hipStream_t s, const bf16_t* A, int64_t lda, const bf16_t* B, int64_t ldb, float* C, int64_t ldc, int M, int N, int K,
             const float* bias, const float* bias2, int flags);
void gemm_hh_shadow(hipStream_t s, const bf16_t* A, int64_t lda, const bf16_t* B, int64_t ldb, float* C, int64_t ldc, bf16_t* Cb, int64_t ldcb,
                    int M, int N, int K);

void conv_forward(hipStream_t s, bool bf16, const float* x, const float* w, const float* bias, float* y, uint8_t* idx,
                  int B, int H, int W, int Cin, int Cout, int ks, int pad, int relu, int pool,
                  const bf16_t* xb = nullptr, const bf16_t* wb = nullptr, bf16_t* yb = nullptr, int profile_tag = 0,
                  const float* bn_save = nullptr, const float* bn_w = nullptr, const float* bn_b = nullptr,
                  double* bn_part = nullptr, int* bn_chunks = nullptr, int* y_bf16 = nullptr);
void bn_eval_prepare(hipStream_t s, const float* rm, const float* rv, float* save, int C);
struct BnBwdFuse { const float* x; const bf16_t* yb; const float* save; double* part; };
void conv_backward_data(hipStream_t s, bool bf16, const float* dy, const float* w, float* dx, int B, int H, int W, int Cin,
                        int Cout, int ks, int pad, const bf16_t* dyb = nullptr, const bf16_t* wtb = nullptr, const float* wtf = nullptr,
                        int* dx16 = nullptr ,
                        const struct BnBwdFuse* bnb = nullptr, int* bnb_chunks = nullptr );
void conv_backward_filter(hipStream_t s, bool bf16, const float* x, const float* dy, float* dw, float* dbias, int B, int H,
                          int W, int Cin, int Cout, int ks, int pad, const bf16_t* xb = nullptr, const bf16_t* dyb = nullptr,
                          float* part = nullptr, size_t part_floats = 0, int profile_tag = 0);
void splitk_reduce(hipStream_t s, const float* part, int ks, size_t n, float* out);

void conv1_forward(hipStream_t s, const float* x, const float* w, const float* bias, float* y, int B, int H, int W,
                   bf16_t* yb = nullptr, uint16_t* route = nullptr);
size_t conv1_route_elems(int B, int H, int W);
void conv_weight_shadows(hipStream_t s, const float* w, bf16_t* wb, bf16_t* wtb, int Cout, int KK, int Cin);
struct ColsumJobs;
void conv1_backward(hipStream_t s, const float* x, const float* w, const float* bias, const float* dyp, float* dw, float* db,
                    int B, int H, int W, float* scratch = nullptr, ColsumJobs* defer = nullptr,
                    const uint16_t* route = nullptr );
void unpool_relu_backward(hipStream_t s, const float* dpooled, const float* pooled, const uint8_t* idx, float* dy, int B,
                          int Ho, int Wo, int C, int pool, bf16_t* dyb = nullptr, float* dbias = nullptr,
                          float* partial = nullptr, const bf16_t* pooledb = nullptr, ColsumJobs* defer = nullptr,
                          const bf16_t* dpooled16 = nullptr );
void bf16_to_f32(hipStream_t s, const bf16_t* src, float* dst, int64_t n);
size_t bn_scratch_bytes(int C);
struct BnSync { int (*allreduce)(void* ctx, void* buf, int64_t count, int dtype, hipStream_t s); void* ctx; };
void bn_relu_forward(hipStream_t s, const float* x, float* y, const float* w, const float* b, float* rm, float* rv,
                     float* save, void* scratch, int64_t rows, int C, int training, int update_running, int tb_rows,
                     bf16_t* yb = nullptr, const BnSync* sync = nullptr, int stats_chunks = 0 ,
                     const bf16_t* xh = nullptr );
void bn_relu_backward(hipStream_t s, const float* x, const float* y, const float* dA, const float* w, const float* save,
                      float* dx, float* dw, float* db, void* scratch, int64_t rows, int C, int tb_rows, bf16_t* dxb = nullptr,
                      const bf16_t* yb = nullptr, float* conv_dbias = nullptr, float* partial = nullptr, const BnSync* sync = nullptr,
                      ColsumJobs* defer = nullptr, const bf16_t* xh = nullptr ,
                      const bf16_t* dAh = nullptr ,
                      int sums_chunks = 0 );
void attention_forward(hipStream_t s, const float* ctx, const float* q, float* a, float* c, int64_t ldc, int B, int T, int Hd,
                       int ctx_div = 1, bf16_t* cb = nullptr, int64_t ldcb = 0, const bf16_t* ctxb = nullptr);
void gates_elem_bwd(hipStream_t s, const EpGatesBwd& ep, int M, int H);
bool attention_dual_ok(int T, int Hd, const bf16_t* ctxb, const bf16_t* ctxab);
void attention_forward_dual(hipStream_t s, const float* h_top, int64_t ldh, float* a, float* c, int64_t ldc, int B, int T, int ctx_div, bf16_t* cb, int64_t ldcb,
                            const bf16_t* ctxb, const bf16_t* ctxab);
void attention_backward_dual(hipStream_t s, const float* a, const float* dc, int64_t lddc, float* ds, float* dq, bf16_t* dqb, float* dh_attn, int B, int T,
                             const bf16_t* ctxb, const bf16_t* ctxab);
void attention_backward(hipStream_t s, const float* ctx, const float* q, const float* a, const float* dc, int64_t lddc,
                        float* ds, float* dq, int B, int T, int Hd, bf16_t* dqb = nullptr, const bf16_t* ctxb = nullptr,
                        const float* cfwd = nullptr, int64_t ldcf = 0);
void attention_dctx(hipStream_t s, const float* a_all, const float* ds_all, const float* dc_all, int64_t lddc,
                    const float* q_all, float* dctx, int L, int B, int T, int Hd);
void logsoftmax_nll(hipStream_t s, const float* logits, int64_t ld, const int32_t* tgt, int64_t tgt_stride_t,
                    int64_t tgt_stride_b, int Bt, float* logp, float* dlogits, float* nll_rows, int64_t rows, int V,
                    float grad_scale);
void sum_to_scalar(hipStream_t s, const float* x, int64_t n, float* out);
void gold_scores(hipStream_t s, const float* nll_rows, float* gold, int L, int B);
struct ZeroList { void* p[16]; size_t bytes[16]; int n = 0;
  void add(void* q, size_t b) { if (q && b && n < 16) { p[n] = q; bytes[n] = b; ++n; } } };
void zero_many(hipStream_t s, const ZeroList& z);
void colsum_accum(hipStream_t s, const float* A, int64_t ld, int64_t rows, int N, float* out, float* out2 = nullptr);
struct ColsumJob { const float* A; int64_t ld, rows; int N; float* out; float* out2; int first, nb, chunks; };
struct ColsumJobs { int n, total; ColsumJob j[8]; };
void colsum_defer(ColsumJobs& g, const float* A, int64_t ld, int64_t rows, int N, float* out, float* out2 = nullptr);
void colsum_flush(hipStream_t s, ColsumJobs& g);
// ... 163 lines not shown
```

### torch-attention-ocr_amd/csrc/ops_gemm.hip

```cpp
#include "ops.h"
#include "stepl.h"

namespace aocr {

static void split_k(int K, int chunk, int& ksplit, int& kper) {
  if (ksplit < 1) ksplit = 1;
  kper = cdiv(cdiv(K, ksplit), chunk) * chunk;
  if (kper < chunk) kper = chunk;
  ksplit = cdiv(K, kper); if (ksplit < 1) ksplit = 1;
}
static thread_local const char* t_trace_fn = nullptr;
struct TraceScope { explicit TraceScope(const char* fn) { t_trace_fn = fn; } ~TraceScope() { t_trace_fn = nullptr; } };
static void trace_launch(const char* kernel, const char* inst, long long M, long long N, long long K) {
  if (t_trace_fn && getenv("AOCR_TRACE")) fprintf(stderr, "[aocr] %s: %s[%s] %lld %lld %lld\n", t_trace_fn, kernel, inst, M, N, K);
}
static void trace_step(int nt, int gates, int waves, int mt, long long M, long long N, long long K) {
  if (!t_trace_fn || !getenv("AOCR_TRACE")) return;
  char inst[32]; snprintf(inst, sizeof inst, "%d,%d,w%d%s", nt, gates, waves, mt == 2 ? ",mt2" : "");
  trace_launch("gemm_step_kernel", inst, M, N, K);
}
template <class AL, class BL, class EP>
static void launch_lds(hipStream_t s, const AL& a, const BL& b, const EP& ep, int M, int N, int K, int ksplit) {
  if (M <= 0 || N <= 0) return;
  int kper; split_k(K, 32, ksplit, kper);
// ... 666 lines not shown
      if (staged && !(halo && getenv("AOCR_HALO8"))) {
        ep.bn_part = bn_part; *bn_chunks = a.rows / 256;
        if (y_bf16 && getenv("AOCR_BN_Y16") && Cout % 4 == 0 && !getenv("AOCR_BN_PARTIAL_OLD")) {
          ep.y16 = reinterpret_cast<bf16_t*>(y); ep.y = nullptr; *y_bf16 = 1; }
      }
    }
    if (dma_eligible(a.rows, Cout, a.K, Cin) && pad == 1 && halo_eligible(a, Cout, 256, 256)) launch_halo<1, 256, 256>(s, ah, bh, ep, a.rows, Cout, profile_tag);
    else if (dma_eligible(a.rows, Cout, a.K, Cin)) launch_dma(s, ah, bh, ep, a.rows, Cout, a.K, profile_tag);
    else if (dma_narrow_eligible(a.rows, Cout, a.K, Cin) || dma_mid_eligible(a.rows, Cout, a.K, Cin)) launch_dma_narrow(s, ah, bh, ep, a.rows, Cout, a.K);
    else if (dma128_eligible(a.rows, Cout, a.K, Cin)) launch_dma128(s, ah, bh, ep, a.rows, Cout, a.K);
    else launch_lds(s, ah, bh, ep, a.rows, Cout, a.K, 1);
  } else {
    launch_conv_fwd(s, bf16, a, make_loadk(w, a.K, Cout, a.K), ep, a.rows, Cout, a.K);
  }
}

void conv_backward_data(hipStream_t s, bool bf16, const float* dy, const float* w, float* dx, int B, int H, int W, int Cin,
                        int Cout, int ks, int pad, const bf16_t* dyb, const bf16_t* wtb, const float* wtf, int* dx16, const BnBwdFuse* bnb, int* bnb_chunks) {
  const TraceScope ts("conv_backward_data");
  const int Ho = H + 2 * pad - ks + 1, Wo = W + 2 * pad - ks + 1;
  LoadConvK a = make_convk(dy, B, Ho, Wo, Cout, ks, -1, pad, H, W, 0);
  EpStore ep = make_store(dx, Cin, a.rows, Cin);
  if (dx16) *dx16 = 0;
  if (bnb_chunks) *bnb_chunks = 0;
  if (bf16 && dyb && wtb) {
    LoadConvKh ah; ah.src = dyb; ah.g = a;
    LoadKh bh; bh.p = wtb; bh.ld = a.K; bh.rows = Cin; bh.K = a.K;
    if (dx16 && dma_eligible(a.rows, Cin, a.K, Cout) && a.rows % 256 == 0 && Cin % 256 == 0 && env_is_1("AOCR_DX16") && !getenv("AOCR_BN_PARTIAL_OLD") && !getenv("AOCR_UNPOOL4")) {
      const char* const so = getenv("AOCR_HALO4_STAGED");
      const bool halo = pad == 1 && halo_eligible(a, Cin, 256, 256);
      if (((so ? atoi(so) : 7) & 1) && !(halo && getenv("AOCR_HALO8"))) { ep.C = nullptr; ep.Cb = reinterpret_cast<bf16_t*>(dx); ep.ldcb = Cin; *dx16 = 1; }
    }
    if (bnb && bnb_chunks && ep.C && dma_eligible(a.rows, Cin, a.K, Cout) && a.rows % 256 == 0 && Cin % 256 == 0 && a.rows / 256 <= 512 && env_is_1("AOCR_BNB_FUSE")) {
      const char* const so = getenv("AOCR_HALO4_STAGED");
      const bool halo = pad == 1 && halo_eligible(a, Cin, 256, 256);
      if (((so ? atoi(so) : 7) & 1) && !(halo && getenv("AOCR_HALO8"))) {
        ep.bnb_x = bnb->x; ep.bnb_yb = bnb->yb; ep.bnb_save = bnb->save; ep.bnb_part = bnb->part; *bnb_chunks = a.rows / 256;
      }
    }
    if (dma_eligible(a.rows, Cin, a.K, Cout) && pad == 1 && halo_eligible(a, Cin, 256, 256)) launch_halo<-1, 256, 256>(s, ah, bh, ep, a.rows, Cin);
    else if (dma_eligible(a.rows, Cin, a.K, Cout)) launch_dma(s, ah, bh, ep, a.rows, Cin, a.K);
    else if (dma_narrow_eligible(a.rows, Cin, a.K, Cout)) launch_dma_narrow(s, ah, bh, ep, a.rows, Cin, a.K);
    else if (dma128_eligible(a.rows, Cin, a.K, Cout)) launch_dma128(s, ah, bh, ep, a.rows, Cin, a.K);
    else launch_lds(s, ah, bh, ep, a.rows, Cin, a.K, 1);
  } else if (wtf) {
    launch_big(s, bf16, a, make_loadk(wtf, a.K, Cin, a.K), ep, a.rows, Cin, a.K, 1);
  } else {
    LoadConvWT b; b.w = w; b.Cin = Cin; b.Cout = Cout; b.KK = ks * ks; b.K = a.K;
    launch_conv_dgrad(s, bf16, a, b, ep, a.rows, Cin, a.K);
  }
}

void conv_backward_filter(hipStream_t s, bool bf16, const float* x, const float* dy, float* dw, float* dbias, int B, int H,
                          int W, int Cin, int Cout, int ks, int pad, const bf16_t* xb, const bf16_t* dyb, float* part, size_t part_floats, int profile_tag) {
  const TraceScope ts("conv_backward_filter");
  const int Ho = H + 2 * pad - ks + 1, Wo = W + 2 * pad - ks + 1;
  const int P = B * Ho * Wo, N = ks * ks * Cin;
  LoadConvXcol b; b.x = x; b.H = H; b.W = W; b.Cin = Cin; b.KW = ks; b.pad = pad; b.Ho = Ho; b.Wo = Wo; b.N = N; b.K = P;
  EpStore ep = make_store(dw, N, Cout, N, nullptr, nullptr, EP_ATOMIC);
  const int ksplit = pick_ksplit(Cout, N, P, bf16, (bf16 && xb && dyb) ? 1024 : 768);
  if (bf16 && xb && dyb) {
    LoadMNh ah; ah.p = dyb; ah.ld = Cout; ah.rows = Cout; ah.K = P;
    LoadConvXcolh bh; bh.x = xb; bh.g = b;
    const int tiles = cdiv(N, 256) * (Cout / 256);
    const int hmt = Cout % 256 == 0 ? 256 : 128;
    const int spr = (W + 31) / 32;
    const bool ragged_ok = W % 32 == 0 || (!env_is_0("AOCR_WGRAD_HALO_RAGGED") && W * 4 >= spr * 32 * 3);
    if (ks == 3 && pad == 1 && ragged_ok && Cout % hmt == 0 && Cin % 32 == 0 && part && !dma_disabled() && !env_is_1("AOCR_NO_WGRAD_HALO") && !getenv("AOCR_WGRAD_ATOMIC") &&
        (dma_forced() || (P >= 8192 && N >= wgrad_halo_min_n()))) {
      const int htiles = (Cin / 32) * (Cout / hmt), S = B * H * spr;
      int ksh = htiles >= 256 ? 1 : 256 / htiles; if (ksh > S) ksh = S;
      { const char* ms = getenv("AOCR_WGRAD_HALO_MINSTEPS"); const int minsteps = ms ? atoi(ms) : 0;
        if (minsteps > 0 && S / ksh < minsteps) ksh = std::max(1, S / minsteps); }
      const int per = cdiv(S, ksh); ksh = cdiv(S, per);
      const size_t mn = (size_t)Cout * N;
      if (mn * ksh <= part_floats) {
#define AOCR_WGH(TAGV, MGV, RGV, IMV, THREADS, MTV) hipLaunchKernelGGL((conv_wgrad_halo_kernel<TAGV, MGV, RGV, IMV>), dim3(htiles * ksh), dim3(THREADS), 0, s, dyb, xb, part, (long long)mn, B, H, W, Cin, Cout, Cin / 32, Cout / MTV, ksh, per, zero_page())
        const bool im = !env_is_1("AOCR_NO_WGRAD_ISSUE_MID");
        { char inst[48]; snprintf(inst, sizeof inst, "%d,%s,%s", hmt, W % 32 ? "ragged" : "whole", im ? "issue_mid" : "no_issue_mid");
          trace_launch("conv_wgrad_halo_kernel", inst, Cout, N, P); }
        if (W % 32) {
          if (hmt == 128) { if (im) AOCR_WGH(0, 2, true, true, 256, 128); else AOCR_WGH(0, 2, true, false, 256, 128); }
          else { if (im) AOCR_WGH(0, 4, true, true, 512, 256); else AOCR_WGH(0, 4, true, false, 512, 256); }
        }
        else if (hmt == 128) { if (im) AOCR_WGH(0, 2, false, true, 256, 128); else AOCR_WGH(0, 2, false, false, 256, 128); }
        else if (profile_tag) { if (im) AOCR_WGH(1, 4, false, true, 512, 256); else AOCR_WGH(1, 4, false, false, 512, 256); }
        else { if (im) AOCR_WGH(0, 4, false, true, 512, 256); else AOCR_WGH(0, 4, false, false, 512, 256); }
#undef AOCR_WGH
        splitk_reduce(s, part, ksh, mn, dw);
        if (dbias) colsum_accum(s, dy, Cout, P, Cout, dbias);
        return;
      }
    }
    if (Cout % 256 == 0 && Cin % 8 == 0 && !dma_disabled() && (dma_forced() || (P >= 8192 && tiles <= 256 && N % 256 == 0 && N >= 2304))) {
      int ks2 = tiles >= 128 ? (tiles >= 200 ? 1 : 2) : 256 / tiles, kper2; split_k(P, 32, ks2, kper2);
      const size_t mn = (size_t)Cout * N;
      float* const slab = (part && ks2 > 1 && mn * ks2 <= part_floats && !getenv("AOCR_WGRAD_ATOMIC")) ? part : nullptr;
      trace_launch("conv_wgrad_dma_kernel", slab ? "slab" : "atomic", Cout, N, P);
      if (profile_tag)
        hipLaunchKernelGGL((conv_wgrad_dma_kernel<EpStore, 256>), dim3(tiles * ks2), dim3(512), 0, s, ah, bh, ep, P, kper2, cdiv(N, 256), Cout / 256, zero_page(), ks2, slab, (long long)mn);
      else
        hipLaunchKernelGGL((conv_wgrad_dma_kernel<EpStore>), dim3(tiles * ks2), dim3(512), 0, s, ah, bh, ep, P, kper2, cdiv(N, 256), Cout / 256, zero_page(), ks2, slab, (long long)mn);
      if (slab) splitk_reduce(s, slab, ks2, mn, dw);
      if (dbias) colsum_accum(s, dy, Cout, P, Cout, dbias);
      return;
    }
    int ks = ksplit, kper; split_k(P, 32, ks, kper);
    const int gx = cdiv(N, 128), gy = cdiv(Cout, 128);
    const size_t mn = (size_t)Cout * N;
    float* const slab = (part && ks > 1 && mn * ks <= part_floats && !getenv("AOCR_WGRAD_ATOMIC")) ? part : nullptr;
    trace_launch("conv_wgrad_tr_kernel", slab ? "slab" : "atomic", Cout, N, P);
    hipLaunchKernelGGL((conv_wgrad_tr_kernel<EpStore>), dim3(gx * gy * ks), dim3(256), 0, s, ah, bh, ep, P, kper, gx, gy, ks, slab, (long long)mn);
    if (slab) splitk_reduce(s, slab, ks, mn, dw);
  } else {
    launch_conv_wgrad(s, bf16, make_loadmn(dy, Cout, Cout, P), b, ep, Cout, N, P, ksplit);
  }
  if (dbias) colsum_accum(s, dy, Cout, P, Cout, dbias);
}

}
```

Before: 53980 image-lines/s.

## Fuse split-K reduction into conv wgrad kernels via per-tile arrival counters

Each split-K wgrad workgroup now bumps a per-tile atomic counter after writing its partial slab, and the last one to arrive sums all partials into dw itself. This removes the separate splitk_reduce launch and its extra pass over the partial buffer for the halo, dma and tr wgrad kernels. Counter regions are zeroed by folding them into existing zero_many batches, with a memset fallback. The cost is a tail of serial reduction work in the last-arriving workgroup of each tile, plus fence and atomic overhead.

```diff
diff --git a/include/aocr.h b/include/aocr.h
--- a/include/aocr.h
+++ b/include/aocr.h
@@ -142,6 +142,9 @@
 int aocr_conv2d_backward_filter(void* stream, int32_t compute, const float* x_dev, const float* dy_dev, float* dw_dev,
                                 float* dbias_dev, int32_t B, int32_t H, int32_t W, int32_t Cin, int32_t Cout,
                                 int32_t ksize, int32_t pad);
+int aocr_conv2d_backward_filter_ws(void* stream, int32_t compute, const float* x_dev, const float* dy_dev, float* dw_dev,
+                                   float* dbias_dev, int32_t B, int32_t H, int32_t W, int32_t Cin, int32_t Cout,
+                                   int32_t ksize, int32_t pad, void* workspace_dev, size_t workspace_bytes, int32_t fused);
 int aocr_unpool_relu_backward(void* stream, const float* dpooled_dev, const float* pooled_dev, const uint8_t* idx_dev,
                               float* dy_dev, int32_t B, int32_t Ho, int32_t Wo, int32_t C, int32_t pool);
 
diff --git a/torch-attention-ocr_amd/aocr/_lib.py b/torch-attention-ocr_amd/aocr/_lib.py
--- a/torch-attention-ocr_amd/aocr/_lib.py
+++ b/torch-attention-ocr_amd/aocr/_lib.py
@@ -130,6 +130,7 @@
     "aocr_conv2d_forward": (C.c_int, [_vp, _i32, _vp, _vp, _vp, _vp, _vp] + [_i32] * 9),
     "aocr_conv2d_backward_data": (C.c_int, [_vp, _i32, _vp, _vp, _vp] + [_i32] * 7),
     "aocr_conv2d_backward_filter": (C.c_int, [_vp, _i32, _vp, _vp, _vp, _vp] + [_i32] * 7),
+    "aocr_conv2d_backward_filter_ws": (C.c_int, [_vp, _i32, _vp, _vp, _vp, _vp] + [_i32] * 7 + [_vp, C.c_size_t, _i32]),
     "aocr_unpool_relu_backward": (C.c_int, [_vp, _vp, _vp, _vp, _vp] + [_i32] * 5),
     "aocr_conv1_forward": (C.c_int, [_vp, _vp, _vp, _vp, _vp, _i32, _i32, _i32]),
     "aocr_conv1_backward": (C.c_int, [_vp, _vp, _vp, _vp, _vp, _vp, _vp, _i32, _i32, _i32]),
diff --git a/torch-attention-ocr_amd/csrc/capi.hip b/torch-attention-ocr_amd/csrc/capi.hip
--- a/torch-attention-ocr_amd/csrc/capi.hip
+++ b/torch-attention-ocr_amd/csrc/capi.hip
@@ -484,7 +484,15 @@
                    m->A6b, 1);
       break;
     case 1:
-      conv_backward_filter(m->s, m->bf16, m->A5, m->G0, m->G1, nullptr, d.B, d.H4, d.W2, 512, 512, 3, 1, m->A5b, m->G0b, m->wg_part, m->wg_part_floats, 1);
+      {
+        int* cnt = nullptr;
+        if (m->wg_cnt) {
+          constexpr int R0 = 6, NR = WG_CNT_REGIONS - R0;
+          if (m->wg_cnt_replay % NR == 0) hipMemsetAsync(m->wg_cnt + (size_t)R0 * WGRAD_TILE_CNT, 0, (size_t)NR * WGRAD_TILE_CNT * sizeof(int), m->s);
+          cnt = m->wg_cnt + (size_t)(R0 + m->wg_cnt_replay % NR) * WGRAD_TILE_CNT; ++m->wg_cnt_replay;
+        }
+        conv_backward_filter(m->s, m->bf16, m->A5, m->G0, m->G1, nullptr, d.B, d.H4, d.W2, 512, 512, 3, 1, m->A5b, m->G0b, m->wg_part, m->wg_part_floats, 1, cnt, WGRAD_TILE_CNT);
+      }
       break;
     case AOCR_PK_CONV1_FWD:
       conv1_forward(s, m->last_images, m->conv[1].w, m->conv[1].b, nullptr, B, d.H, d.W, m->A1b, m->route1_valid ? m->route1 : nullptr);
@@ -586,6 +594,28 @@
   conv_backward_filter((hipStream_t)stream, compute == AOCR_COMPUTE_BF16, x_dev, dy_dev, dw_dev, dbias_dev, B, H, W, Cin, Cout, ksize, pad);
   return check_launch("aocr_conv2d_backward_filter");
 }
+int aocr_conv2d_backward_filter_ws(void* stream, int32_t compute, const float* x_dev, const float* dy_dev, float* dw_dev, float* dbias_dev,
+                                   int32_t B, int32_t H, int32_t W, int32_t Cin, int32_t Cout, int32_t ksize, int32_t pad, void* workspace_dev,
+                                   size_t workspace_bytes, int32_t fused) {
+  REQUIRE(x_dev && dy_dev && dw_dev && Cin % 16 == 0 && Cout % 16 == 0 && B > 0 && H > 0 && W > 0 && ksize > 0 && pad >= 0, "bad arguments");
+  REQUIRE(compute == AOCR_COMPUTE_BF16, "the split-K filter gradient is a bf16-mode path");
+  const int Ho = H + 2 * pad - ksize + 1, Wo = W + 2 * pad - ksize + 1;
+  REQUIRE(Ho > 0 && Wo > 0, "kernel larger than the padded map");
+  auto r256 = [](size_t b) { return (b + 255) & ~(size_t)255; };
+  const size_t cnt_bytes = (size_t)WGRAD_TILE_CNT * sizeof(int), xb_bytes = r256((size_t)B * H * W * Cin * 2), dyb_bytes = r256((size_t)B * Ho * Wo * Cout * 2);
+  REQUIRE(workspace_dev && ((uintptr_t)workspace_dev & 255) == 0, "workspace must be 256-byte aligned");
+  REQUIRE(workspace_bytes >= cnt_bytes + xb_bytes + dyb_bytes, "workspace of %zu bytes: the counters and the bf16 operand images alone take %zu", workspace_bytes, cnt_bytes + xb_bytes + dyb_bytes);
+  unsigned char* const w = (unsigned char*)workspace_dev;
+  bf16_t* const xb = reinterpret_cast<bf16_t*>(w + cnt_bytes); bf16_t* const dyb = reinterpret_cast<bf16_t*>(w + cnt_bytes + xb_bytes);
+  float* const part = reinterpret_cast<float*>(w + cnt_bytes + xb_bytes + dyb_bytes);
+  const size_t part_floats = (workspace_bytes - (cnt_bytes + xb_bytes + dyb_bytes)) / sizeof(float);
+  hipStream_t s = (hipStream_t)stream;
+  copy2d_bf16(s, x_dev, Cin, xb, Cin, B * H * W, Cin);
+  copy2d_bf16(s, dy_dev, Cout, dyb, Cout, B * Ho * Wo, Cout);
+  conv_backward_filter(s, true, x_dev, dy_dev, dw_dev, dbias_dev, B, H, W, Cin, Cout, ksize, pad, xb, dyb, part_floats ? part : nullptr, part_floats, 0,
+                       fused ? reinterpret_cast<int*>(w) : nullptr, WGRAD_TILE_CNT);
+  return check_launch("aocr_conv2d_backward_filter_ws");
+}
 int aocr_unpool_relu_backward(void* stream, const float* dpooled_dev, const float* pooled_dev, const uint8_t* idx_dev, float* dy_dev,
                               int32_t B, int32_t Ho, int32_t Wo, int32_t C, int32_t pool) {
   REQUIRE(dpooled_dev && pooled_dev && idx_dev && dy_dev && (pool == 1 || pool == 2) && C % 4 == 0, "bad arguments");
diff --git a/torch-attention-ocr_amd/csrc/mfma_gemm.h b/torch-attention-ocr_amd/csrc/mfma_gemm.h
--- a/torch-attention-ocr_amd/csrc/mfma_gemm.h
+++ b/torch-attention-ocr_amd/csrc/mfma_gemm.h
@@ -1910,20 +1910,59 @@
     }
 }
 
+template <int NT>
+__device__ __forceinline__ void wgrad_finish_tile(const float* part, long long pstride, int ks, int* cnt, float* dw, int64_t ld, int row0, int rows, int col0,
+                                                  int nrun, int run4, int64_t runstride, int* flag) {
+  typedef float f4 __attribute__((ext_vector_type(4)));
+  asm volatile("s_waitcnt vmcnt(0)" ::: "memory");
+  __syncthreads();
+  if (threadIdx.x == 0) {
+    __builtin_amdgcn_fence(__ATOMIC_RELEASE, "agent");
+    asm volatile("s_waitcnt vmcnt(0)" ::: "memory");
+    const int t = __hip_atomic_fetch_add(cnt, 1, __ATOMIC_RELAXED, __HIP_MEMORY_SCOPE_AGENT);
+    if (t == ks - 1) { __builtin_amdgcn_fence(__ATOMIC_ACQUIRE, "agent"); asm volatile("s_waitcnt vmcnt(0)" ::: "memory"); }
+    *flag = t;
+  }
+  __syncthreads();
+  if (*flag != ks - 1) return;
+  const int rq = nrun * run4, total = rows * rq;
+  const size_t ps4 = (size_t)pstride / 4;
+  for (int i = threadIdx.x; i < total; i += NT) {
+    const int row = i / rq, c = i - row * rq, u = c / run4, j = c - u * run4;
+    const int64_t off = (int64_t)(row0 + row) * ld + col0 + u * runstride + 4 * j;
+    const f4* p = reinterpret_cast<const f4*>(part + off);
+    f4 acc = *reinterpret_cast<const f4*>(dw + off);
+    int z = 0;
+    for (; z + 8 <= ks; z += 8) {
+      f4 v[8];
+#pragma unroll
+      for (int k = 0; k < 8; ++k) v[k] = p[(size_t)(z + k) * ps4];
+#pragma unroll
+      for (int k = 0; k < 8; ++k) acc += v[k];
+    }
+    for (; z < ks; ++z) acc += p[(size_t)z * ps4];
+    *reinterpret_cast<f4*>(dw + off) = acc;
+  }
+}
+
 template <class EP>
-__global__ __launch_bounds__(256, 4) void conv_wgrad_tr_kernel(LoadMNh a, LoadConvXcolh b, EP ep, int K, int kper, int gx, int gy, int gz, float* part, long long pstride) {
+__global__ __launch_bounds__(256, 4) void conv_wgrad_tr_kernel(LoadMNh a, LoadConvXcolh b, EP ep, int K, int kper, int gx, int gy, int gz, float* part, long long pstride, int* cnt = nullptr) {
   __shared__ __attribute__((aligned(16))) unsigned char lds[2][2][32 * TR_PITCH];
   const int nwg = gx * gy * gz, orig = blockIdx.x;
   const int q8 = nwg >> 3, r8 = nwg & 7, xcd = orig & 7;
   const int lin = (xcd < r8 ? xcd * (q8 + 1) : r8 * (q8 + 1) + (xcd - r8) * q8) + (orig >> 3);
   const int zsp = lin / (gx * gy), bid = lin - zsp * (gx * gy);
   const int kbeg = zsp * kper;
+  float* const dw = ep.C;
   if (part) { ep.C = part + (size_t)zsp * pstride; ep.flags &= ~8 ; }
-  tr_tile(a, b, ep, (bid / gx) * 128, (bid % gx) * 128, kbeg, min(K, kbeg + kper), lds);
+  const int m_blk = (bid / gx) * 128, n_blk = (bid % gx) * 128;
+  tr_tile(a, b, ep, m_blk, n_blk, kbeg, min(K, kbeg + kper), lds);
+  if (part && cnt)
+    wgrad_finish_tile<256>(part, pstride, gz, cnt + bid, dw, ep.ldc, m_blk, min(128, ep.M - m_blk), n_blk, 1, min(128, ep.N - n_blk) >> 2, 0, reinterpret_cast<int*>(&lds[0][0][0]));
 }
 
 template <class EP, int ABL = 0>
-__global__ __launch_bounds__(512, 1) void conv_wgrad_dma_kernel(LoadMNh a, LoadConvXcolh b, EP ep, int K, int kper, int gx, int gy, const bf16_t* zero, int gz, float* part, long long pstride) {
+__global__ __launch_bounds__(512, 1) void conv_wgrad_dma_kernel(LoadMNh a, LoadConvXcolh b, EP ep, int K, int kper, int gx, int gy, const bf16_t* zero, int gz, float* part, long long pstride, int* cnt = nullptr) {
   __shared__ __attribute__((aligned(1024))) unsigned char lds[4 * 32768];
   const int nwg = gx * gy * gz, orig = blockIdx.x;
   const int q8 = nwg >> 3, r8 = nwg & 7, xcd = orig & 7;
@@ -1931,6 +1970,7 @@
   const int zsp = lin / (gx * gy), bid = lin - zsp * (gx * gy);
   const int m_blk = (bid / gx) * 256, n_blk = (bid % gx) * 256;
   const int kbeg = zsp * kper, kend = min(K, kbeg + kper);
+  float* const dw = ep.C;
   if (part) { ep.C = part + (size_t)zsp * pstride; ep.flags &= ~8 ; }
   const int nk = kend > kbeg ? (kend - kbeg + 31) >> 5 : 0;
   const int tid = threadIdx.x, lane = tid & 63, wave = __builtin_amdgcn_readfirstlane(tid >> 6);
@@ -2034,6 +2074,7 @@
   if constexpr (std::is_same<EP, EpStore>::value && ABL == 0) {
     if (part && !ep.flags && !ep.bias && !ep.bias2 && !ep.C1 && !ep.Cb && !ep.dg && m_blk + 256 <= ep.M && n_blk + 256 <= ep.N) {
       tile256_store_f32<2, 512>(ep.C, ep.ldc, nullptr, false, acc, lds, m_blk, n_blk, wm, wn, r, h, tid);
+      if (cnt) wgrad_finish_tile<512>(part, pstride, gz, cnt + bid, dw, ep.ldc, m_blk, 256, n_blk, 1, 64, 0, reinterpret_cast<int*>(lds));
       return;
     }
   }
@@ -2048,6 +2089,8 @@
         for (int i = 0; i < 4; ++i) v[ni][i] = acc[mi][ni][4 * qq + i];
       ep.template quad<2>(m0 + 32 * mi + 8 * qq + 4 * h, n0 + r, 32, v);
     }
+  if constexpr (std::is_same<EP, EpStore>::value && ABL == 0)
+    if (part && cnt) wgrad_finish_tile<512>(part, pstride, gz, cnt + bid, dw, ep.ldc, m_blk, min(256, ep.M - m_blk), n_blk, 1, min(256, ep.N - n_blk) >> 2, 0, reinterpret_cast<int*>(lds));
 }
 
 struct WgDmaProblem { const bf16_t* A; const bf16_t* B; long long lda, ldb; int M, N, K, gx, tiles, ks, kper, first; float* part; float* C; long long ldc; long long f4first; };
@@ -2165,7 +2208,7 @@
 template <int TAG = 0, int MG = 4, bool RG = false, bool IM = false>
 __global__ __launch_bounds__(128 * MG, 1)
 void conv_wgrad_halo_kernel(const bf16_t* __restrict__ dy, const bf16_t* __restrict__ x, float* __restrict__ part, long long pstride,
-                            int nimg, int H, int W, int Cin, int Cout, int gx, int gy, int gz, int segs_per, const bf16_t* zero) {
+                            int nimg, int H, int W, int Cin, int Cout, int gx, int gy, int gz, int segs_per, const bf16_t* zero, int* cnt = nullptr, float* dw = nullptr) {
   constexpr int MT = 64 * MG, NWV = 2 * MG, AROW = MT * 2, RPP = 1024 / AROW, LPR = 64 / RPP;
   constexpr int BOFF = 32 * AROW, SLOT = BOFF + 8192, NS = 6, PW = 34, HPW = 8 / NWV;
   __shared__ __attribute__((aligned(1024))) unsigned char lds[NWV * 20480 > NS * SLOT ? NWV * 20480 : NS * SLOT];
@@ -2326,6 +2369,7 @@
   };
   if (tg == 0) body(std::integral_constant<int, 0>{}); else body(std::integral_constant<int, 1>{});
 #undef AOCR_TRH
+  if (cnt) wgrad_finish_tile<128 * MG>(part, pstride, gz, cnt + bid, dw, ldw, m_blk, MT, cchunk * 32, 9, 8, Cin, reinterpret_cast<int*>(lds));
 }
 
 template <class AL, class BL, class EP> struct GroupProblem { AL a; BL b; EP ep; int K, kper, gx, ksplit, first; };
diff --git a/torch-attention-ocr_amd/csrc/model.h b/torch-attention-ocr_amd/csrc/model.h
--- a/torch-attention-ocr_amd/csrc/model.h
+++ b/torch-attention-ocr_amd/csrc/model.h
@@ -43,6 +43,7 @@
 
 }
 
+constexpr int WG_CNT_REGIONS = 16;
 struct aocr_model {
   aocr_config cfg;
   hipStream_t s;
@@ -90,6 +91,7 @@
   float *attn_hist = nullptr, *sc_hist = nullptr;
   void* sgd_scratch;
   float* wg_part = nullptr; size_t wg_part_floats = 0;
+  int* wg_cnt = nullptr; bool wg_cnt_clean = false; int wg_cnt_replay = 0;
 
   std::vector<aocr::ShadowJob> shadow_host;
   aocr::ShadowJob* shadow_dev; int shadow_tiles;
diff --git a/torch-attention-ocr_amd/csrc/model.hip b/torch-attention-ocr_amd/csrc/model.hip
--- a/torch-attention-ocr_amd/csrc/model.hip
+++ b/torch-attention-ocr_amd/csrc/model.hip
@@ -157,6 +157,7 @@
   m->trie_loc[0] = a.get<int32_t>(R); m->trie_loc[1] = a.get<int32_t>(R);
   m->sgd_scratch = a.get<char>(sgd_scratch_bytes());
   m->wg_part_floats = m->bf16 ? (size_t)20 << 20 : 0;       m->wg_part = m->wg_part_floats ? a.get<float>(m->wg_part_floats) : nullptr;
+  m->wg_cnt = m->wg_part_floats ? a.get<int>((size_t)WG_CNT_REGIONS * WGRAD_TILE_CNT) : nullptr;
   if (m->bf16 && He % 64 == 0 && He <= 512) {
     m->cl_xbytes = m->Le * enc_cluster_xbuf_bytes((int)B, (int)He); m->cl_pbytes = m->Le * enc_cluster_pbuf_bytes((int)B, (int)He);
     m->cl_xbuf = a.get<unsigned long long>(m->cl_xbytes / 8); m->cl_pbuf = a.get<unsigned long long>(m->cl_pbytes / 8);
@@ -364,6 +365,9 @@
   hipStream_t sw = ws ? m->side : s;
   const bool wg_after = ws && env_on("AOCR_CNN_WGRAD_AFTER_DGRAD");
   if (!ws) Gb[1] = Gb[0];
+  if (m->wg_cnt && !m->wg_cnt_clean) hipMemsetAsync(m->wg_cnt, 0, (size_t)6 * WGRAD_TILE_CNT * sizeof(int), s);
+  m->wg_cnt_clean = false;
+  auto wcnt = [&](int layer) { return m->wg_cnt ? m->wg_cnt + (size_t)(layer - 2) * WGRAD_TILE_CNT : nullptr; };
   auto map_ready = [&]() { if (ws) { hipEventRecord(m->cw_map[gp], s); hipStreamWaitEvent(sw, m->cw_map[gp], 0); } };
   auto wgrad_done = [&]() { if (ws) hipEventRecord(m->cw_done[gp], sw); };
   auto next_map = [&]() { if (ws) { gp ^= 1; hipStreamWaitEvent(s, m->cw_done[gp], 0); } };
@@ -376,17 +380,17 @@
   prof_mark(m, AOCR_PROF_BN); bn_relu_backward(s, m->Y7, m->X, m->dX, m->bn[7].w, m->bn[7].save, bf ? nullptr : G0, m->bn[7].dw, m->bn[7].db, m->bn_scratch,
                    (int64_t)B * d.T, 512, B, Gb[gp], bf ? m->Xb : nullptr, bf ? m->conv[7].db : nullptr, bf ? slab(0) : nullptr, bsync, defer);
   if (stop == 1) { if (defer) colsum_flush(s, cj); return; }
-  { auto W = [&]() { prof_mark(m, AOCR_PROF_CONV_WGRAD); conv_backward_filter(sw, bf, m->A6, G0, m->conv[7].dw, bf ? nullptr : m->conv[7].db, B, d.H6, d.W2, 512, 512, 2, 0, m->A6b, Gb[gp], m->wg_part, m->wg_part_floats); };
+  { auto W = [&]() { prof_mark(m, AOCR_PROF_CONV_WGRAD); conv_backward_filter(sw, bf, m->A6, G0, m->conv[7].dw, bf ? nullptr : m->conv[7].db, B, d.H6, d.W2, 512, 512, 2, 0, m->A6b, Gb[gp], m->wg_part, m->wg_part_floats, 0, wcnt(7), WGRAD_TILE_CNT); };
     auto D = [&]() { prof_mark(m, AOCR_PROF_CONV_DGRAD); conv_backward_data(s, bf, G0, m->conv[7].w, G1, B, d.H6, d.W2, 512, 512, 2, 0, Gb[gp], m->wtb[7], m->wtf[7], bf ? &g16 : nullptr); };
     if (wg_after) { D(); map_ready(); W(); wgrad_done(); } else { map_ready(); W(); wgrad_done(); D(); } }
   next_map(); prof_mark(m, AOCR_PROF_POOL_CONV1); unpool_relu_backward(s, G1, m->A6, m->idx6, bf ? nullptr : G0, B, d.H4, d.W2, 512, 2, Gb[gp], bf ? m->conv[6].db : nullptr, bf ? slab(1) : nullptr, bf ? m->A6b : nullptr, defer, g16 ? G1h : nullptr);
   if (stop == 2) { if (defer) colsum_flush(s, cj); return; }
-  { auto W = [&]() { prof_mark(m, AOCR_PROF_CONV_WGRAD); conv_backward_filter(sw, bf, m->A5, G0, m->conv[6].dw, bf ? nullptr : m->conv[6].db, B, d.H4, d.W2, 512, 512, 3, 1, m->A5b, Gb[gp], m->wg_part, m->wg_part_floats); };
+  { auto W = [&]() { prof_mark(m, AOCR_PROF_CONV_WGRAD); conv_backward_filter(sw, bf, m->A5, G0, m->conv[6].dw, bf ? nullptr : m->conv[6].db, B, d.H4, d.W2, 512, 512, 3, 1, m->A5b, Gb[gp], m->wg_part, m->wg_part_floats, 0, wcnt(6), WGRAD_TILE_CNT); };
     auto D = [&]() { prof_mark(m, AOCR_PROF_CONV_DGRAD); { const BnBwdFuse bf5{m->Y5, m->A5b, m->bn[5].save, (double*)m->bn_scratch}; conv_backward_data(s, bf, G0, m->conv[6].w, G1, B, d.H4, d.W2, 512, 512, 3, 1, Gb[gp], m->wtb[6], m->wtf[6], bf ? &g16 : nullptr, (bf && !m->y16[1]) ? &bf5 : nullptr, &bnbc); } };
     if (wg_after) { D(); map_ready(); W(); wgrad_done(); } else { map_ready(); W(); wgrad_done(); D(); } }
   next_map(); prof_mark(m, AOCR_PROF_BN); bn_relu_backward(s, m->Y5, m->A5, G1, m->bn[5].w, m->bn[5].save, bf ? nullptr : G0, m->bn[5].dw, m->bn[5].db, m->bn_scratch,
                    (int64_t)B * d.H4 * d.W2, 512, 0, Gb[gp], bf ? m->A5b : nullptr, bf ? m->conv[5].db : nullptr, bf ? slab(2) : nullptr, bsync, defer, m->y16[1] ? reinterpret_cast<const bf16_t*>(m->Y5) : nullptr, g16 ? G1h : nullptr, bnbc); bnbc = 0;
-  { auto W = [&]() { prof_mark(m, AOCR_PROF_CONV_WGRAD); conv_backward_filter(sw, bf, m->A4, G0, m->conv[5].dw, bf ? nullptr : m->conv[5].db, B, d.H4, d.W2, 256, 512, 3, 1, m->A4b, Gb[gp], m->wg_part, m->wg_part_floats); };
+  { auto W = [&]() { prof_mark(m, AOCR_PROF_CONV_WGRAD); conv_backward_filter(sw, bf, m->A4, G0, m->conv[5].dw, bf ? nullptr : m->conv[5].db, B, d.H4, d.W2, 256, 512, 3, 1, m->A4b, Gb[gp], m->wg_part, m->wg_part_floats, 0, wcnt(5), WGRAD_TILE_CNT); };
     auto D = [&]() { prof_mark(m, AOCR_PROF_CONV_DGRAD); conv_backward_data(s, bf, G0, m->conv[5].w, G1, B, d.H4, d.W2, 256, 512, 3, 1, Gb[gp], m->wtb[5], m->wtf[5], bf ? &g16 : nullptr); };
     if (wg_after) { D(); map_ready(); W(); wgrad_done(); } else { map_ready(); W(); wgrad_done(); }
   if (defer) colsum_flush(s, cj);
@@ -394,16 +398,16 @@
   else hipEventRecord(m->grad_ev[2], s);
     if (!wg_after) D(); }
   next_map(); prof_mark(m, AOCR_PROF_POOL_CONV1); unpool_relu_backward(s, G1, m->A4, m->idx4, bf ? nullptr : G0, B, d.H2, d.W2, 256, 2, Gb[gp], bf ? m->conv[4].db : nullptr, bf ? slab(3) : nullptr, bf ? m->A4b : nullptr, defer, g16 ? G1h : nullptr);
-  { auto W = [&]() { prof_mark(m, AOCR_PROF_CONV_WGRAD); conv_backward_filter(sw, bf, m->A3, G0, m->conv[4].dw, bf ? nullptr : m->conv[4].db, B, d.H2, d.W2, 256, 256, 3, 1, m->A3b, Gb[gp], m->wg_part, m->wg_part_floats); };
+  { auto W = [&]() { prof_mark(m, AOCR_PROF_CONV_WGRAD); conv_backward_filter(sw, bf, m->A3, G0, m->conv[4].dw, bf ? nullptr : m->conv[4].db, B, d.H2, d.W2, 256, 256, 3, 1, m->A3b, Gb[gp], m->wg_part, m->wg_part_floats, 0, wcnt(4), WGRAD_TILE_CNT); };
     auto D = [&]() { prof_mark(m, AOCR_PROF_CONV_DGRAD); { const BnBwdFuse bf3{m->Y3, m->A3b, m->bn[3].save, (double*)m->bn_scratch}; conv_backward_data(s, bf, G0, m->conv[4].w, G1, B, d.H2, d.W2, 256, 256, 3, 1, Gb[gp], m->wtb[4], m->wtf[4], bf ? &g16 : nullptr, (bf && !m->y16[0]) ? &bf3 : nullptr, &bnbc); } };
     if (wg_after) { D(); map_ready(); W(); wgrad_done(); } else { map_ready(); W(); wgrad_done(); D(); } }
   next_map(); prof_mark(m, AOCR_PROF_BN); bn_relu_backward(s, m->Y3, m->A3, G1, m->bn[3].w, m->bn[3].save, bf ? nullptr : G0, m->bn[3].dw, m->bn[3].db, m->bn_scratch,
                    (int64_t)B * d.H2 * d.W2, 256, 0, Gb[gp], bf ? m->A3b : nullptr, bf ? m->conv[3].db : nullptr, bf ? slab(4) : nullptr, bsync, defer, m->y16[0] ? reinterpret_cast<const bf16_t*>(m->Y3) : nullptr, g16 ? G1h : nullptr, bnbc); bnbc = 0;
-  { auto W = [&]() { prof_mark(m, AOCR_PROF_CONV_WGRAD); conv_backward_filter(sw, bf, m->A2, G0, m->conv[3].dw, bf ? nullptr : m->conv[3].db, B, d.H2, d.W2, 128, 256, 3, 1, m->A2b, Gb[gp], m->wg_part, m->wg_part_floats); };
+  { auto W = [&]() { prof_mark(m, AOCR_PROF_CONV_WGRAD); conv_backward_filter(sw, bf, m->A2, G0, m->conv[3].dw, bf ? nullptr : m->conv[3].db, B, d.H2, d.W2, 128, 256, 3, 1, m->A2b, Gb[gp], m->wg_part, m->wg_part_floats, 0, wcnt(3), WGRAD_TILE_CNT); };
     auto D = [&]() { prof_mark(m, AOCR_PROF_CONV_DGRAD); conv_backward_data(s, bf, G0, m->conv[3].w, G1, B, d.H2, d.W2, 128, 256, 3, 1, Gb[gp], m->wtb[3], m->wtf[3]); };
     if (wg_after) { D(); map_ready(); W(); wgrad_done(); } else { map_ready(); W(); wgrad_done(); D(); } }
   next_map(); prof_mark(m, AOCR_PROF_POOL_CONV1); unpool_relu_backward(s, G1, m->A2, m->idx2, bf ? nullptr : G0, B, d.H1, d.W1, 128, 1, Gb[gp], bf ? m->conv[2].db : nullptr, bf ? slab(5) : nullptr, bf ? m->A2b : nullptr, defer);
-  { auto W = [&]() { prof_mark(m, AOCR_PROF_CONV_WGRAD); conv_backward_filter(sw, bf, m->A1, G0, m->conv[2].dw, bf ? nullptr : m->conv[2].db, B, d.H1, d.W1, 64, 128, 3, 1, m->A1b, Gb[gp], m->wg_part, m->wg_part_floats); };
+  { auto W = [&]() { prof_mark(m, AOCR_PROF_CONV_WGRAD); conv_backward_filter(sw, bf, m->A1, G0, m->conv[2].dw, bf ? nullptr : m->conv[2].db, B, d.H1, d.W1, 64, 128, 3, 1, m->A1b, Gb[gp], m->wg_part, m->wg_part_floats, 0, wcnt(2), WGRAD_TILE_CNT); };
     auto D = [&]() { prof_mark(m, AOCR_PROF_CONV_DGRAD); conv_backward_data(s, bf, G0, m->conv[2].w, G1, B, d.H1, d.W1, 64, 128, 3, 1, Gb[gp], m->wtb[2], m->wtf[2]); };
     if (wg_after) { D(); map_ready(); W(); wgrad_done(); } else { map_ready(); W(); wgrad_done(); D(); } }
   prof_mark(m, AOCR_PROF_POOL_CONV1); conv1_backward(s, images, m->conv[1].w, m->conv[1].b, G1, m->conv[1].dw, m->conv[1].db, B, d.H, d.W,
@@ -465,6 +469,11 @@
   return true;
 }
 static void reserve_epochs(aocr_model* m, unsigned n) { if (m->cl_epoch + n + 1 >= (1u << 20)) { m->cl_epoch = (1u << 20); (void)next_epoch(m); } }
+
+static void wg_cnt_zero(aocr_model* m, ZeroList& zl) {
+  if (!m->wg_cnt || zl.n >= 16) return;
+  zl.add(m->wg_cnt, (size_t)6 * WGRAD_TILE_CNT * sizeof(int)); m->wg_cnt_clean = true;
+}
 
 static void encoder_forward_pipe(aocr_model* m, const Dims& d, int C, int clG, int clRT, int clGroups) {
   hipStream_t s0 = m->s;
@@ -477,6 +486,7 @@
       zl.add(m->ecs[dir][l], slot * sizeof(float)); zl.add(m->ecs[dir][l] + (size_t)(T + 1) * slot, slot * sizeof(float));
       zl.add(m->ehs_b[dir][l], slot * sizeof(bf16_t)); zl.add(m->ehs_b[dir][l] + (size_t)(T + 1) * slot, slot * sizeof(bf16_t));
     }
+    if (l == 0) wg_cnt_zero(m, zl);
     zero_many(s0, zl);
   }
   for (int dir = 0; dir < 2; ++dir) {
@@ -561,6 +571,7 @@
       }
     }
     prof_mark(m, AOCR_PROF_OTHER);
+    if (l == 0) wg_cnt_zero(m, zl);
     zero_many(s, zl);
     prof_mark(m, AOCR_PROF_ENC_SEQ);
     const bool top = l == m->Le - 1;
diff --git a/torch-attention-ocr_amd/csrc/ops.h b/torch-attention-ocr_amd/csrc/ops.h
--- a/torch-attention-ocr_amd/csrc/ops.h
+++ b/torch-attention-ocr_amd/csrc/ops.h
@@ -101,7 +101,9 @@
                         const struct BnBwdFuse* bnb = nullptr, int* bnb_chunks = nullptr );
 void conv_backward_filter(hipStream_t s, bool bf16, const float* x, const float* dy, float* dw, float* dbias, int B, int H,
                           int W, int Cin, int Cout, int ks, int pad, const bf16_t* xb = nullptr, const bf16_t* dyb = nullptr,
-                          float* part = nullptr, size_t part_floats = 0, int profile_tag = 0);
+                          float* part = nullptr, size_t part_floats = 0, int profile_tag = 0,
+                          int* tile_cnt = nullptr, int tile_cnt_n = 0);
+constexpr int WGRAD_TILE_CNT = 1024;
 void splitk_reduce(hipStream_t s, const float* part, int ks, size_t n, float* out);
 
 void conv1_forward(hipStream_t s, const float* x, const float* w, const float* bias, float* y, int B, int H, int W,
diff --git a/torch-attention-ocr_amd/csrc/ops_gemm.hip b/torch-attention-ocr_amd/csrc/ops_gemm.hip
--- a/torch-attention-ocr_amd/csrc/ops_gemm.hip
+++ b/torch-attention-ocr_amd/csrc/ops_gemm.hip
@@ -742,8 +742,10 @@
 }
 
 void conv_backward_filter(hipStream_t s, bool bf16, const float* x, const float* dy, float* dw, float* dbias, int B, int H,
-                          int W, int Cin, int Cout, int ks, int pad, const bf16_t* xb, const bf16_t* dyb, float* part, size_t part_floats, int profile_tag) {
+                          int W, int Cin, int Cout, int ks, int pad, const bf16_t* xb, const bf16_t* dyb, float* part, size_t part_floats, int profile_tag,
+                          int* tile_cnt, int tile_cnt_n) {
   const TraceScope ts("conv_backward_filter");
+  if (tile_cnt && env_is_1("AOCR_NO_WGRAD_FUSED_SUM")) tile_cnt = nullptr;
   const int Ho = H + 2 * pad - ks + 1, Wo = W + 2 * pad - ks + 1;
   const int P = B * Ho * Wo, N = ks * ks * Cin;
   LoadConvXcol b; b.x = x; b.H = H; b.W = W; b.Cin = Cin; b.KW = ks; b.pad = pad; b.Ho = Ho; b.Wo = Wo; b.N = N; b.K = P;
@@ -765,9 +767,10 @@
       const int per = cdiv(S, ksh); ksh = cdiv(S, per);
       const size_t mn = (size_t)Cout * N;
       if (mn * ksh <= part_floats) {
-#define AOCR_WGH(TAGV, MGV, RGV, IMV, THREADS, MTV) hipLaunchKernelGGL((conv_wgrad_halo_kernel<TAGV, MGV, RGV, IMV>), dim3(htiles * ksh), dim3(THREADS), 0, s, dyb, xb, part, (long long)mn, B, H, W, Cin, Cout, Cin / 32, Cout / MTV, ksh, per, zero_page())
+        int* const fcnt = (tile_cnt && htiles <= tile_cnt_n) ? tile_cnt : nullptr;
+#define AOCR_WGH(TAGV, MGV, RGV, IMV, THREADS, MTV) hipLaunchKernelGGL((conv_wgrad_halo_kernel<TAGV, MGV, RGV, IMV>), dim3(htiles * ksh), dim3(THREADS), 0, s, dyb, xb, part, (long long)mn, B, H, W, Cin, Cout, Cin / 32, Cout / MTV, ksh, per, zero_page(), fcnt, dw)
         const bool im = !env_is_1("AOCR_NO_WGRAD_ISSUE_MID");
-        { char inst[48]; snprintf(inst, sizeof inst, "%d,%s,%s", hmt, W % 32 ? "ragged" : "whole", im ? "issue_mid" : "no_issue_mid");
+        { char inst[64]; snprintf(inst, sizeof inst, "%d,%s,%s%s", hmt, W % 32 ? "ragged" : "whole", im ? "issue_mid" : "no_issue_mid", fcnt ? ",fused_sum" : "");
           trace_launch("conv_wgrad_halo_kernel", inst, Cout, N, P); }
         if (W % 32) {
           if (hmt == 128) { if (im) AOCR_WGH(0, 2, true, true, 256, 128); else AOCR_WGH(0, 2, true, false, 256, 128); }
@@ -777,7 +780,7 @@
         else if (profile_tag) { if (im) AOCR_WGH(1, 4, false, true, 512, 256); else AOCR_WGH(1, 4, false, false, 512, 256); }
         else { if (im) AOCR_WGH(0, 4, false, true, 512, 256); else AOCR_WGH(0, 4, false, false, 512, 256); }
 #undef AOCR_WGH
-        splitk_reduce(s, part, ksh, mn, dw);
+        if (!fcnt) splitk_reduce(s, part, ksh, mn, dw);
         if (dbias) colsum_accum(s, dy, Cout, P, Cout, dbias);
         return;
       }
@@ -786,12 +789,13 @@
       int ks2 = tiles >= 128 ? (tiles >= 200 ? 1 : 2) : 256 / tiles, kper2; split_k(P, 32, ks2, kper2);
       const size_t mn = (size_t)Cout * N;
       float* const slab = (part && ks2 > 1 && mn * ks2 <= part_floats && !getenv("AOCR_WGRAD_ATOMIC")) ? part : nullptr;
-      trace_launch("conv_wgrad_dma_kernel", slab ? "slab" : "atomic", Cout, N, P);
+      int* const fcnt = (slab && tile_cnt && tiles <= tile_cnt_n && !profile_tag) ? tile_cnt : nullptr;
+      trace_launch("conv_wgrad_dma_kernel", fcnt ? "slab,fused_sum" : slab ? "slab" : "atomic", Cout, N, P);
       if (profile_tag)
         hipLaunchKernelGGL((conv_wgrad_dma_kernel<EpStore, 256>), dim3(tiles * ks2), dim3(512), 0, s, ah, bh, ep, P, kper2, cdiv(N, 256), Cout / 256, zero_page(), ks2, slab, (long long)mn);
       else
-        hipLaunchKernelGGL((conv_wgrad_dma_kernel<EpStore>), dim3(tiles * ks2), dim3(512), 0, s, ah, bh, ep, P, kper2, cdiv(N, 256), Cout / 256, zero_page(), ks2, slab, (long long)mn);
-      if (slab) splitk_reduce(s, slab, ks2, mn, dw);
+        hipLaunchKernelGGL((conv_wgrad_dma_kernel<EpStore>), dim3(tiles * ks2), dim3(512), 0, s, ah, bh, ep, P, kper2, cdiv(N, 256), Cout / 256, zero_page(), ks2, slab, (long long)mn, fcnt);
+      if (slab && !fcnt) splitk_reduce(s, slab, ks2, mn, dw);
       if (dbias) colsum_accum(s, dy, Cout, P, Cout, dbias);
       return;
     }
@@ -799,9 +803,10 @@
     const int gx = cdiv(N, 128), gy = cdiv(Cout, 128);
     const size_t mn = (size_t)Cout * N;
     float* const slab = (part && ks > 1 && mn * ks <= part_floats && !getenv("AOCR_WGRAD_ATOMIC")) ? part : nullptr;
-    trace_launch("conv_wgrad_tr_kernel", slab ? "slab" : "atomic", Cout, N, P);
-    hipLaunchKernelGGL((conv_wgrad_tr_kernel<EpStore>), dim3(gx * gy * ks), dim3(256), 0, s, ah, bh, ep, P, kper, gx, gy, ks, slab, (long long)mn);
-    if (slab) splitk_reduce(s, slab, ks, mn, dw);
+    int* const fcnt = (slab && tile_cnt && gx * gy <= tile_cnt_n) ? tile_cnt : nullptr;
+    trace_launch("conv_wgrad_tr_kernel", fcnt ? "slab,fused_sum" : slab ? "slab" : "atomic", Cout, N, P);
+    hipLaunchKernelGGL((conv_wgrad_tr_kernel<EpStore>), dim3(gx * gy * ks), dim3(256), 0, s, ah, bh, ep, P, kper, gx, gy, ks, slab, (long long)mn, fcnt);
+    if (slab && !fcnt) splitk_reduce(s, slab, ks, mn, dw);
   } else {
     launch_conv_wgrad(s, bf16, make_loadmn(dy, Cout, Cout, P), b, ep, Cout, N, P, ksplit);
   }
```

After: 46140 image-lines/s. 0.855x the previous value.
